# ai4r/Gesture-Generation-from-Trimodal-Context

Measured on AMD Instinct MI355X. Metric: training clips/sec (34-frame, 27-dim pose), post-warm-up GAN iteration, higher is better.
Workload: dtype f32; 1 GPU; multimodal_context GAN training iteration (BASELINE.json configs[1]), epoch > loss_warmup; batch_per_gpu=128, global_batch=128, frames=34, pose_dim=27, audio_samples=36267, n_words=20000, hipgraph=True, parallelism=dp1

## Files before the change

### gesture-generation-from-trimodal-context_amd/_lib.py

```python
import ctypes as C
import os

_HERE = os.path.dirname(os.path.abspath(__file__))
LIB_PATH = os.environ.get("TG_LIB_PATH") or os.path.join(_HERE, "libtrimodal_hip.so")


class Window(C.Structure):
    _fields_ = [("ptr", C.c_void_p), ("batch_stride", C.c_int64), ("row_stride", C.c_int64), ("rows_in", C.c_int32),
                ("rows_out", C.c_int32), ("row_step", C.c_int32), ("shift", C.c_int32), ("dil", C.c_int32),
                ("cw", C.c_int32), ("K", C.c_int32)]


P, I32, I64, F32, U32 = C.c_void_p, C.c_int32, C.c_int64, C.c_float, C.c_uint32
WP = C.POINTER(Window)


class NtProblem(C.Structure):
    _fields_ = [("A", Window), ("Bw", P), ("ldb", I64), ("b_seg_k", I32), ("reserved", I32), ("b_seg_stride", I64), ("bias", P), ("C", P),
                ("c_batch_stride", I64), ("c_row_stride", I64), ("c_rows_out", I32), ("M", I32), ("N", I32), ("act_slope", F32),
                ("accumulate", I32), ("out_scale", P), ("b_planes", P), ("b_plane_stride", I64), ("b_rows", I32), ("b_row0", I32),
                ("gate", P), ("res", P), ("C2", P), ("res_slope", F32), ("drop_site", U32), ("drop_state", P), ("drop_index0", I64),
                ("drop_p", F32), ("reserved4", I32), ("b_planes_kind", I32), ("reserved5", I32), ("b_inv_scale", P), ("a_row_scale", P), ("a_rowmax", P), ("c_rowmax", P), ("c2_rowmax", P), ("a_rowmax_rows", I32), ("reserved6", I32)]


class TnProblem(C.Structure):
    _fields_ = [("dY", P), ("ldy", I64), ("A", Window), ("dW", P), ("ldw", I64), ("M", I32), ("N", I32), ("out_kw", I32), ("reserved", I32),
                ("dbias", P), ("ws", P), ("ws_floats", I64), ("y_colmax", P), ("a_colmax", P)]


class AeStepArgs(C.Structure):
    _fields_ = [("x", P), ("params", P), ("grads", P), ("off", I32 * 44), ("running_mean", P * 8), ("running_var", P * 8),
                ("num_batches_tracked", P * 8), ("ws", P), ("ws_bytes", I64), ("loss", P), ("recon", P), ("feat", P), ("step", P), ("B", I32),
                ("bn_eps", F32), ("momentum", F32), ("last_phase", I32), ("adam_m", P), ("adam_v", P), ("lr", F32), ("beta1", F32), ("beta2", F32), ("adam_eps", F32)]


MAX_GROUP = 8

SIGNATURES = {
    "tg_gemm_nt": [WP, P, I64, P, P, I64, I64, I32, I32, I32, F32, I32, P],
    "tg_gemm_nt_group": [C.POINTER(NtProblem), I32, P],
    "tg_gemm_tn_group": [C.POINTER(TnProblem), I32, P],
    "tg_ae_train_step": [C.POINTER(AeStepArgs), P],
    "tg_split3_planes": [P, I64, I32, I32, P, I32, I64, P],
    "tg_split2h_planes": [P, I64, I32, I32, P, I32, I64, P, P],
    "tg_split2h_planes_tcat": [P, P, I32, I32, P, I32, I64, P, P],
    "tg_win_row_absmax": [WP, I32, P, P],
    "tg_h2_row_scales": [WP, I32, P, P, P],
    "tg_absmax_rows_cols": [P, I64, I32, I32, I32, P, P, P],
    "tg_gemm_tn": [P, I64, WP, P, I64, I32, I32, I32, P, P, I64, P],
    "tg_colsum": [P, I64, I32, I32, P, I32, P],
    "tg_gru_forward": [P, I64, P, P, P, P, P, P, I64, I32, I32, I32, P],
    "tg_gru_backward": [P, P, P, I64, P, P, P, P, I64, P, I32, I32, I32, P],
    "tg_gru_h64_forward": [P, I64, P, P, P, P, P, P, I64, P, P, I32, I32, P],
    "tg_gru_h64_backward": [P, P, P, P, I64, P, P, P, P, I64, I32, I32, P],
    "tg_gru_forward_cluster": [P, I64, P, P, P, P, P, P, I64, P, P, P, I64, I32, I32, I32, P],
    "tg_gru_forward_cluster_rows": [P, I64, P, P, P, P, P, P, I64, P, P, P, I64, I32, I32, I32, I32, I32, P],
    "tg_gru_forward_vec": [P, I64, P, P, P, P, P, P, I64, I32, I32, I32, P],
    "tg_gru_vec1_supported": [I32, I32, P],
    "tg_gru_forward_vec1": [P, P, P, P, P, I64, I32, I32, I32, P],
    "tg_gru_vec_const_supported": [I32, I32, I32, P],
    "tg_gru_forward_vec_const": [P, I64, P, P, P, P, P, P, I64, I32, I32, I32, I32, P],
    "tg_gru_backward_cluster": [P, P, P, P, I64, P, P, P, P, I64, P, I64, I32, I32, I32, P],
    "tg_gru_backward_cluster_stats": [P, P, P, P, I64, P, P, P, P, I64, P, I64, I32, I32, I32, P, I64, P, P, P],
    "tg_bn_train_stats": [P, I32, I32, I32, P, P, P, P, P, P, F32, F32, I32, P],
    "tg_bn_eval_stats": [P, P, I32, F32, P, P, P],
    "tg_bn_train_fused": [P, P, I32, I32, I32, P, P, P, P, P, P, P, F32, F32, F32, I32, P],
    "tg_bn_apply": [P, P, I32, I32, I32, P, P, P, P, F32, P],
    "tg_bn2_train": [P, P, I32, I32, I32, P, I64, P, P, P, P, P, P, P, F32, F32, F32, I32, P],
    "tg_bn2_backward": [P, P, P, I32, I32, I32, P, P, P, P, F32, P, I64, P, P, P],
    "tg_bn_backward": [P, P, P, I32, I32, P, P, P, P, F32, P, P, P, P],
    "tg_wav_front_stats": [P, I64, I32, I32, P, P, I32, I32, I32, P, I64, P, P, P, P, P, P, F32, F32, I32, P],
    "tg_wav_front_apply": [P, I64, I32, I32, P, P, I32, I32, I32, P, P, P, P, F32, P, P, P],
    "tg_wav_front_backward": [P, P, P, I64, I32, I32, P, P, I32, I32, I32, P, P, P, P, F32, P, I64, P, P, P, P, P],
    "tg_wav_front_backward_fused": [P, I32, P, P, P, I64, I32, I32, P, P, I32, I32, I32, P, P, P, P, F32, P, I64, P, P, P, P, P],
    "tg_speaker_fwd": [P, P, I32, P, P, P, P, P, P, P, P, P, P, P, P, I32, P, I64, I32, P, U32, P],
    "tg_speaker_bwd": [P, P, P, P, P, P, P, P, I32, P, P, P, P, P, P, P, P, P, P, I32, P],
    "tg_wav_conv2_wgrad": [P, P, I32, I32, I32, P, I64, P, P, P],
    "tg_out_mlp_compose": [P, P, P, P, I32, I32, I32, I32, P, P, P, P],
    "tg_out_mlp_param_grads": [P, P, P, P, P, I32, I32, I32, I32, P, P, P, P, P],
    "tg_zero": [P, I64, P],
    "tg_permute3_batch": [P, I32, I32, P],
    "tg_add_relu": [P, P, P, I64, P],
    "tg_act_mask_bwd": [P, P, P, F32, P, I64, P],
    "tg_act_mask_bwd2": [P, P, P, P, F32, P, P, I64, P],
    "tg_embed_gather_drop": [P, P, P, I32, I32, I32, F32, P, U32, P],
    "tg_tcn_fwd_fused": [P, P, I64, I32, P, C.POINTER(P), P, P, P, U32, F32, I32, I32, I32, I32, P, P, P, I32, I32, P, I64, P],
    "tg_d_preconv_bwd": [P] * 26 + [I32, P, I64, I32, I32, P],
    "tg_d_preconv_fwd": [P] * 27 + [I64, I32, I32, F32, F32, P],
    "tg_iter_head": [P, P, P, P, P, P, I64, I32, I32, I32, I32, I32, P, P, P, P, I32, P, U32, P, P, P],
    "tg_act_mask_bwd_drop": [P, P, F32, P, U32, I64, F32, P, I64, P],
    "tg_act_mask_bwd2_drop": [P, P, P, F32, P, U32, I64, F32, P, P, I64, P],
    "tg_mul": [P, P, P, I64, P],
    "tg_axpy": [P, P, F32, I32, I64, P],
    "tg_copy2d": [P, I64, P, I64, I32, I32, I32, P],
    "tg_repeat_rows": [P, I64, P, I64, I32, I32, I32, P],
    "tg_sum_rows": [P, I64, P, I64, I32, I32, I32, I32, P],
    "tg_add_halves": [P, P, I32, I32, P],
    "tg_sum_parts": [P, I64, I32, P, I64, P],
    "tg_narrow8_pair": [P, P, P, P, P, I32, I32, P],
    "tg_dup_halves": [P, P, I32, I32, P],
    "tg_make_pre_seq": [P, P, I32, I32, I32, I32, P],
    "tg_embed_gather": [P, P, P, I32, I32, I32, P],
    "tg_assemble_batch": [P, P, P, P, P, P, P, P, P, P, I32, I32, I32, I32, I32, I32, P, P, P, P, P],
    "tg_embed_scatter_add": [P, P, P, I32, I32, I32, P],
    "tg_permute3": [P, P, I32, I32, I32, I32, I32, I32, P],
    "tg_conv_dgrad_pack": [P, P, I32, I32, I32, I32, P],
    "tg_weight_norm_fwd": [P, P, P, I32, I32, I32, P],
    "tg_weight_norm_fwd_batch": [I32, C.POINTER(P), C.POINTER(P), C.POINTER(P), C.POINTER(P), I32, I32, I32, P],
    "tg_weight_norm_bwd": [P, P, P, P, P, I32, I32, I32, P],
    "tg_weight_norm_bwd_batch": [I32, C.POINTER(P), C.POINTER(P), C.POINTER(P), C.POINTER(P), C.POINTER(P), I32, I32, I32, P],
    "tg_rng_advance": [P, P],
    "tg_iter_begin": [P, P, P, P, P],
    "tg_dropout_mask": [P, I64, F32, P, U32, P],
    "tg_dropout_apply": [P, P, P, I64, F32, P, U32, P],
    "tg_normal": [P, I64, P, U32, P],
    "tg_randperm": [P, I32, P, U32, P],
    "tg_gather_i64": [P, P, P, I32, P],
    "tg_reparam_fwd": [P, P, P, P, I64, P],
    "tg_reparam_bwd": [P, P, P, P, P, I64, P],
    "tg_gan_d_loss": [P, P, I32, P, P, P, P],
    "tg_gan_g_loss": [P, P, P, P, P, P, P, P, I32, I32, I32, F32, F32, F32, F32, I32, P, P, P, P, P, P, P],
    "tg_d_head_fwd": [P, P, P, P, P, P, P, P, I32, I32, I32, P],
    "tg_d_head_bwd": [P, P, P, P, P, P, P, P, P, P, I32, I32, I32, P],
    "tg_d_head_step": [P] * 17 + [I32, I32, F32, F32, I32, I32, P],
    "tg_l1_mean": [P, P, I64, P, P],
    "tg_sigmoid": [P, P, I64, P],
    "tg_sigmoid_bwd": [P, P, P, I64, P],
    "tg_window_blend": [P, P, I32, I32, I32, I32, P],
    "tg_window_stage": [P, P, P, P, P, P, I32, I32, I32, I32, P, P, P],
    "tg_spec_stage": [P, P, P, P, P, I32, I32, I32, I32, P, P],
    "tg_utterance_finish": [P, I64, I32, I32, P, I32, I32, I32, I32, P, P, P, P, I64, P],
    "tg_pose_metrics": [P, P, P, I32, I32, I32, P, P],
    "tg_ae_loss": [P, P, I32, I32, I32, P, P, P],
    "tg_counter_inc": [P, P],
    "tg_adam_step": [P, P, P, P, I64, F32, F32, F32, F32, P, P],
    "tg_conv2d_fwd": [P, I32, P, P, P] + [I32] * 12 + [P],
    "tg_conv2d_dgrad": [P, P, P, I32] + [I32] * 12 + [P],
    "tg_conv2d_wgrad_ws_bytes": [I32] * 12 + [P],
    "tg_conv2d_wgrad": [P, P, I32, P, I32, P, I64] + [I32] * 12 + [P],
    "tg_s2g_rows_interp": [P, P, I32, I32, I32, I32, I32, I32, P],
    "tg_s2g_rows_interp_bwd": [P, P, I32, I32, I32, I32, I32, I32, P],
    "tg_s2g_up_add": [P, P, P, I32, I32, I32, I32, P],
    "tg_s2g_up_add_bwd": [P, P, I32, I32, I32, I32, I32, P],
    "tg_s2g_diff": [P, P, I32, I32, I32, P],
    "tg_s2g_diff_bwd": [P, P, I32, I32, I32, I32, P],
    "tg_s2g_mse_const": [P, I64, F32, F32, P, P, P],
    "tg_s2g_l1_grad": [P, P, P, I64, P],
    "tg_logmel_query": [I32, I32, P],
    "tg_logmel": [P, I64, I32, I32, I32, P, I64, P, I64, P, I32, P],
    "tg_pose_resample": [P, I64, I32, P, I64, I32, P, I64, P],
    "tg_clip_windows": [P, I64, I32, P, I64, I32, I32, P, I64, P, P, P, P, P],
# ... 115 lines not shown
```

### gesture-generation-from-trimodal-context_amd/csrc/common.hpp

```cpp
#pragma once
#include <hip/hip_runtime.h>
#include <stdint.h>
#include <stdio.h>
#include <string.h>

#include "../../include/trimodal_hip.h"

typedef float f32x4 __attribute__((ext_vector_type(4)));

namespace tg {

void set_error(const char* fmt, ...);

inline int check_launch(const char* what) {
    hipError_t e = hipGetLastError();
    if (e != hipSuccess) {
        set_error("%s: %s", what, hipGetErrorString(e));
        return 1;
    }
    return 0;
}

#define TG_REQUIRE(cond, ...)              \
    do {                                   \
        if (!(cond)) {                     \
            tg::set_error(__VA_ARGS__);    \
            return 2;                      \
        }                                  \
    } while (0)

extern "C" int tg_get_deterministic(void);
inline bool deterministic() { return tg_get_deterministic() != 0; }

inline bool aligned16(const void* p) { return (reinterpret_cast<uintptr_t>(p) & 15u) == 0; }

inline int cdiv(int64_t a, int64_t b) { return (int)((a + b - 1) / b); }

int zero_async(void* p, size_t bytes, hipStream_t s);

inline int ew_grid(int64_t n, int block = 256, int per_thread = 4) {
    int64_t b = (n + (int64_t)block * per_thread - 1) / ((int64_t)block * per_thread);
    if (b < 1) b = 1;
    if (b > 2048) b = 2048;
    return (int)b;
}

struct Win {
    const float* ptr;
    long bs, rs;
    int rows_in, rows_out, step, shift, dil, cw, K;
};

inline Win to_win(const tg_window* w) {
    Win d;
    d.ptr = w->ptr; d.bs = w->batch_stride; d.rs = w->row_stride; d.rows_in = w->rows_in; d.rows_out = w->rows_out;
    d.step = w->row_step; d.shift = w->shift; d.dil = w->dil; d.cw = w->cw; d.K = w->K;
    return d;
}

constexpr int TG_MAX_GROUP = 8;

struct NtProb {
    Win A;
    const float* Bw;
    long ldb;
    long b_seg_stride;
    int b_seg_k;
    const float* bias;
    const float* mul;
    const uint64_t* drop_state;
    long drop_index0;
    unsigned drop_site;
    float drop_p;
    float* C;
    long cbs, crs;
    int cR, M, N;
    float slope;
    int accumulate;
    int n_nt;
    int vec_c;
    const float* gate;
    const float* res;
    float* C2;
    float res_slope;
    unsigned a_bytes, b_bytes;
    const __bf16* Bpl;
    long bpl_plane;
    int b_slab_rows, b_row0;
    const float* a_scale;
    const float* a_rmax;
    int a_rmax_div;
    const float* b_inv;
    int h2;
    float* c_rmax;
    float* c2_rmax;
};

struct NtGroup {
    int n;
    int wg_begin[TG_MAX_GROUP + 1];
    NtProb p[TG_MAX_GROUP];
};

struct TnProb {
    const float* dY;
    long ldy;
    Win A;
    float* dW;
    long ldw;
    int M, N, rows_per_split, out_kw;
    float* partial;
    float* dbias;
    int vec_y, vec_a, n_nt, n_kt;
    unsigned a_bytes, y_bytes;
    const float* y_cmax;
    const float* a_cmax;
};

struct TnGroup {
    int n;
    int wg_begin[TG_MAX_GROUP + 1];
    TnProb p[TG_MAX_GROUP];
};

template <typename G>
__device__ __forceinline__ int group_find(const G& g, int bid) {
    int i = 0;
#pragma unroll
    for (int q = 1; q < TG_MAX_GROUP; ++q) i += (q < g.n && bid >= g.wg_begin[q]) ? 1 : 0;
    return i;
}

__device__ __forceinline__ int xcd_chunked_id(int bid, int nwg) {
    const int q = nwg >> 3, r = nwg & 7, xcd = bid & 7, pos = bid >> 3;
    return (xcd < r ? xcd * (q + 1) : r * (q + 1) + (xcd - r) * q) + pos;
}

__device__ __forceinline__ float act_fn(float x, float slope) { return x >= 0.f ? x : x * slope; }
__device__ __forceinline__ float sigmoidf_(float x) { return 1.f / (1.f + expf(-x)); }
__device__ __forceinline__ float gate_exp_neg(float x) { return __builtin_amdgcn_exp2f(x * -1.44269504088896341f); }
__device__ __forceinline__ float gate_sigmoid(float x) { return __builtin_amdgcn_rcpf(1.f + gate_exp_neg(x)); }
__device__ __forceinline__ float gate_tanh(float x) {
    const float e = gate_exp_neg(2.f * fabsf(x));
    return copysignf((1.f - e) * __builtin_amdgcn_rcpf(1.f + e), x);
}

__device__ __forceinline__ void split3_bits(float x, unsigned& hi, unsigned& mid, unsigned& lo) {
    hi = __float_as_uint(x) & 0xffff0000u;
    const float r = x - __uint_as_float(hi);
    mid = __float_as_uint(r) & 0xffff0000u;
    lo = __float_as_uint(r - __uint_as_float(mid));
}
__device__ __forceinline__ unsigned pack_hi16(unsigned first, unsigned second) { return __builtin_amdgcn_perm(second, first, 0x07060302u); }

__device__ __host__ __forceinline__ long plane_tiled_off(long r, int c, int rows) { return ((long)(c >> 5) * (rows + 1) + r) * 32 + (c & 31); }

typedef _Float16 tg_f16x2 __attribute__((ext_vector_type(2)));
typedef _Float16 tg_f16x8 __attribute__((ext_vector_type(8)));
__device__ __host__ __forceinline__ int h2_exp_of_bits(unsigned absmax_bits) {
    const int e = (int)((absmax_bits & 0x7fffffffu) >> 23);
    return e < 32 ? 32 : (e > 250 ? 250 : e);
}
__device__ __forceinline__ float h2_scale_of_exp(int e) { return __uint_as_float((unsigned)(268 - e) << 23); }
__device__ __forceinline__ float h2_inv_of_exp(int e) { return __uint_as_float((unsigned)(e - 14) << 23); }
__device__ __forceinline__ float h2_inv_of_scale(float s) { return __uint_as_float(0x7f000000u - __float_as_uint(s)); }
__device__ __forceinline__ void h2_split2(float a, float b, unsigned& hi, unsigned& lo) {
    const tg_f16x2 h = {(_Float16)a, (_Float16)b};
    const float ha = (float)h[0], hb = (float)h[1];
    const tg_f16x2 l = {(_Float16)(a - ha), (_Float16)(b - hb)};
    hi = __builtin_bit_cast(unsigned, h);
    lo = __builtin_bit_cast(unsigned, l);
}
__device__ __forceinline__ unsigned wave_max_u32(unsigned v) {
#pragma unroll
    for (int o = 32; o >= 1; o >>= 1) { const unsigned w = (unsigned)__shfl_xor((int)v, o, 64); v = v > w ? v : w; }
    return v;
}

// ... 32 lines not shown
```

### gesture-generation-from-trimodal-context_amd/csrc/gemm.hip

```cpp
#include <stdlib.h>

#include <type_traits>
#include <utility>

#include "operand_split.hpp"

namespace tg {

template <bool VEC>
__device__ __forceinline__ void load_nt_frags(const Win& A, const long (&a_off)[2], const int (&a_r)[2], const bool (&a_ok)[2],
                                              const float* const (&b_ptr)[2], const bool (&b_ok)[2], int k, int kk, int c,
                                              f32x4 (&fa)[2], f32x4 (&fb)[2]) {
    const int K = A.K;
    if (VEC) {
        const bool inb = k < K;
#pragma unroll
        for (int mt = 0; mt < 2; ++mt) {
            const int sr = a_r[mt] + kk * A.dil;
            const bool ok = a_ok[mt] && inb && sr >= 0 && sr < A.rows_in;
            f32x4 z = {0.f, 0.f, 0.f, 0.f};
            fa[mt] = ok ? *reinterpret_cast<const f32x4*>(A.ptr + a_off[mt] + (long)sr * A.rs + c) : z;
        }
#pragma unroll
        for (int nt = 0; nt < 2; ++nt) {
            f32x4 z = {0.f, 0.f, 0.f, 0.f};
            fb[nt] = (b_ok[nt] && inb) ? *reinterpret_cast<const f32x4*>(b_ptr[nt] + k) : z;
        }
    } else {
#pragma unroll
        for (int v = 0; v < 4; ++v) {
            const int kv = k + v;
            const bool inb = kv < K;
            const int kkv = inb ? kv / A.cw : 0;
            const int cv = kv - kkv * A.cw;
#pragma unroll
            for (int mt = 0; mt < 2; ++mt) {
                const int sr = a_r[mt] + kkv * A.dil;
                const bool ok = a_ok[mt] && inb && sr >= 0 && sr < A.rows_in;
                fa[mt][v] = ok ? A.ptr[a_off[mt] + (long)sr * A.rs + cv] : 0.f;
            }
#pragma unroll
            for (int nt = 0; nt < 2; ++nt) fb[nt][v] = (b_ok[nt] && inb) ? b_ptr[nt][kv] : 0.f;
        }
    }
}

template <bool VEC, int WM, int WN, int NT_RING, int KS = 1>
__global__ __launch_bounds__(256) void gemm_nt_kernel(const NtGroup g) {
    static_assert(KS == 1 || (KS == 4 && WM == 1 && WN == 1 && VEC), "K split: one tile per workgroup, vectorised path");
    const int pi = group_find(g, blockIdx.x);
    const NtProb& pr = g.p[pi];
    const Win A = pr.A;
    const float* __restrict__ Bw = pr.Bw;
    const long ldb = pr.ldb;
    const float* __restrict__ bias = pr.bias;
    const float* __restrict__ mul = pr.mul;
    float* __restrict__ C = pr.C;
    const long cbs = pr.cbs, crs = pr.crs;
    const int cR = pr.cR, M = pr.M, N = pr.N, accumulate = pr.accumulate, n_nt = pr.n_nt;
    const float slope = pr.slope;
    const int lane = threadIdx.x & 63;
    const int wave = threadIdx.x >> 6;
    const int wm = KS > 1 ? 0 : wave / WN, wn = KS > 1 ? 0 : wave % WN;
    const int r16 = lane & 15, kq = lane >> 4;
    const int lid = xcd_chunked_id(blockIdx.x - g.wg_begin[pi], g.wg_begin[pi + 1] - g.wg_begin[pi]);
    const int m_base = (lid / n_nt) * (WM * 32) + wm * 32;
    const int n_base = (lid % n_nt) * (WN * 32) + wn * 32;
    if (m_base >= M || n_base >= N) return;
    const int kslice = KS > 1 ? ((A.K + 16 * KS - 1) / (16 * KS)) * 16 : A.K;
    const int K_beg = KS > 1 ? wave * kslice : 0;
    const int K = KS > 1 ? (A.K < K_beg + kslice ? A.K : K_beg + kslice) : A.K;

    long a_off[2];
    int a_r[2];
    bool a_ok[2];
#pragma unroll
    for (int mt = 0; mt < 2; ++mt) {
        const int m = m_base + mt * 16 + r16;
        a_ok[mt] = m < M;
        const int mm = a_ok[mt] ? m : 0;
        const int b = mm / A.rows_out;
        const int r = mm - b * A.rows_out;
        a_off[mt] = (long)b * A.bs;
        a_r[mt] = r * A.step + A.shift;
    }
    const float* b_ptr[2];
    bool b_ok[2];
#pragma unroll
    for (int nt = 0; nt < 2; ++nt) {
        const int n = n_base + nt * 16 + r16;
        b_ok[nt] = n < N;
        b_ptr[nt] = Bw + (long)(b_ok[nt] ? n : 0) * ldb;
    }

    f32x4 acc[2][2];
#pragma unroll
    for (int i = 0; i < 2; ++i)
#pragma unroll
        for (int j = 0; j < 2; ++j) acc[i][j] = f32x4{0.f, 0.f, 0.f, 0.f};

    if constexpr (VEC) {
        constexpr int R = NT_RING;
        int k = K_beg + 4 * kq;
        int kk = k / A.cw, c = k - (k / A.cw) * A.cw;
        f32x4 ra[R][2], rb[R][2];
        unsigned rm[R];
        auto load = [&](auto set_c) {
            constexpr int j = decltype(set_c)::value;
            const bool inb = k < K;
            unsigned m = 0u;
#pragma unroll
            for (int mt = 0; mt < 2; ++mt) {
                const int sr = a_r[mt] + kk * A.dil;
                const bool ok = a_ok[mt] && inb && sr >= 0 && sr < A.rows_in;
                ra[j][mt] = *reinterpret_cast<const f32x4*>(ok ? A.ptr + a_off[mt] + (long)sr * A.rs + c : A.ptr);
                m |= ok ? (1u << mt) : 0u;
            }
#pragma unroll
            for (int nt = 0; nt < 2; ++nt) {
                const bool ok = b_ok[nt] && inb;
                rb[j][nt] = *reinterpret_cast<const f32x4*>(ok ? b_ptr[nt] + k : Bw);
                m |= ok ? (4u << nt) : 0u;
            }
            rm[j] = m;
            k += 16;
            c += 16;
            while (c >= A.cw) { c -= A.cw; ++kk; }
        };
        static_for<R>([&](auto j) { load(j); });
        for (int k0 = K_beg; k0 < K; k0 += 16 * R) {
            static_for<R>([&](auto jc) {
                constexpr int j = decltype(jc)::value;
                {
                    const f32x4 z = {0.f, 0.f, 0.f, 0.f};
                    f32x4 fa[2], fb[2];
#pragma unroll
                    for (int i = 0; i < 2; ++i) {
                        fa[i] = (rm[j] >> i) & 1u ? ra[j][i] : z;
                        fb[i] = (rm[j] >> (2 + i)) & 1u ? rb[j][i] : z;
                    }
#pragma unroll
                    for (int v = 0; v < 4; ++v)
#pragma unroll
                        for (int mt = 0; mt < 2; ++mt)
#pragma unroll
                            for (int nt = 0; nt < 2; ++nt)
                                acc[mt][nt] = __builtin_amdgcn_mfma_f32_16x16x4f32(fa[mt][v], fb[nt][v], acc[mt][nt], 0, 0, 0);
                    if constexpr (R >= 8) { if (k0 + 16 * R < K) load(jc); }
                    else load(jc);
                }
            });
        }
    } else {
        int k = 4 * kq;
        f32x4 fa[2], fb[2], na[2], nb[2];
        load_nt_frags<VEC>(A, a_off, a_r, a_ok, b_ptr, b_ok, k, 0, k, fa, fb);
        for (int k0 = 0; k0 < K; k0 += 16) {
            const bool more = k0 + 16 < K;
            if (more) {
                k += 16;
                load_nt_frags<VEC>(A, a_off, a_r, a_ok, b_ptr, b_ok, k, 0, k, na, nb);
            }
#pragma unroll
            for (int v = 0; v < 4; ++v)
#pragma unroll
                for (int mt = 0; mt < 2; ++mt)
#pragma unroll
                    for (int nt = 0; nt < 2; ++nt)
                        acc[mt][nt] = __builtin_amdgcn_mfma_f32_16x16x4f32(fa[mt][v], fb[nt][v], acc[mt][nt], 0, 0, 0);
            if (more) {
#pragma unroll
                for (int i = 0; i < 2; ++i) { fa[i] = na[i]; fb[i] = nb[i]; }
            }
        }
    }

    if constexpr (KS > 1) {
        __shared__ f32x4 red[KS - 1][4][64];
        if (wave > 0) {
#pragma unroll
            for (int mt = 0; mt < 2; ++mt)
#pragma unroll
                for (int nt = 0; nt < 2; ++nt) red[wave - 1][mt * 2 + nt][lane] = acc[mt][nt];
        }
        __syncthreads();
        if (wave > 0) return;
#pragma unroll
        for (int q = 0; q < KS - 1; ++q)
#pragma unroll
            for (int mt = 0; mt < 2; ++mt)
#pragma unroll
                for (int nt = 0; nt < 2; ++nt) acc[mt][nt] += red[q][mt * 2 + nt][lane];
    }

    long off[2][4][2];
    bool okc[2][4][2];
    float bv[2] = {0.f, 0.f}, mv[2][4][2], cv[2][4][2];
#pragma unroll
    for (int nt = 0; nt < 2; ++nt) {
        const int col = n_base + nt * 16 + r16;
        if (bias) bv[nt] = bias[col < N ? col : 0];
    }
#pragma unroll
    for (int mt = 0; mt < 2; ++mt)
#pragma unroll
        for (int i = 0; i < 4; ++i) {
            const int row = m_base + mt * 16 + kq * 4 + i;
            const int rr = row < M ? row : 0;
            const int cb = rr / cR;
            const int cr = rr - cb * cR;
#pragma unroll
            for (int nt = 0; nt < 2; ++nt) {
                const int col = n_base + nt * 16 + r16;
                okc[mt][i][nt] = row < M && col < N;
                off[mt][i][nt] = okc[mt][i][nt] ? (long)cb * cbs + (long)cr * crs + col : 0;
                if (mul) mv[mt][i][nt] = mul[off[mt][i][nt]];
                if (accumulate) cv[mt][i][nt] = C[off[mt][i][nt]];
            }
        }
#pragma unroll
    for (int mt = 0; mt < 2; ++mt)
#pragma unroll
        for (int i = 0; i < 4; ++i)
#pragma unroll
            for (int nt = 0; nt < 2; ++nt) {
                float v = act_fn(acc[mt][nt][i] + bv[nt], slope);
                if (mul) v *= mv[mt][i][nt];
                if (accumulate) v += cv[mt][i][nt];
                if (okc[mt][i][nt]) C[off[mt][i][nt]] = v;
            }
}

template <int TM, int TN, int BK = 16>
__global__ __launch_bounds__(256) void gemm_nt_big_kernel(const NtGroup g) {
    const int pi = group_find(g, blockIdx.x);
    const NtProb& pr = g.p[pi];
    const Win A = pr.A;
    const float* __restrict__ Bw = pr.Bw;
    const long ldb = pr.ldb, b_seg_stride = pr.b_seg_stride;
    const int b_seg_k = pr.b_seg_k;
    const float* __restrict__ bias = pr.bias;
    const float* __restrict__ mul = pr.mul;
    float* __restrict__ C = pr.C;
    const long cbs = pr.cbs, crs = pr.crs;
    const int cR = pr.cR, M = pr.M, N = pr.N, accumulate = pr.accumulate, n_nt = pr.n_nt;
    const float slope = pr.slope;
    constexpr int BM = 32 * TM, BN = 32 * TN;
    constexpr int PPR = BK / 4;
    constexpr int RPP = 256 / PPR;
    constexpr int NPA = (BM + RPP - 1) / RPP;
    constexpr int NPB = (BN + RPP - 1) / RPP;
    constexpr int LD = BK + 4;
    __shared__ __attribute__((aligned(16))) float as[2][BM][LD];
    __shared__ __attribute__((aligned(16))) float bs[2][BN][LD];
    const int t = threadIdx.x;
    const int lane = t & 63, wave = t >> 6;
    const int wm = wave >> 1, wn = wave & 1;
    const int r16 = lane & 15, kq = lane >> 4;
    const int lid = xcd_chunked_id(blockIdx.x - g.wg_begin[pi], g.wg_begin[pi + 1] - g.wg_begin[pi]);
    const int m0 = (lid / n_nt) * BM, n0 = (lid % n_nt) * BN;
    if (m0 >= M) return;
    const int K = A.K;

    const int srow = t / PPR, sk = 4 * (t % PPR);
    long a_off[NPA];
    int a_r[NPA];
    bool a_ok[NPA];
#pragma unroll
    for (int i = 0; i < NPA; ++i) {
        const int m = m0 + srow + RPP * i;
        a_ok[i] = (srow + RPP * i < BM) && m < M;
        const int mm = a_ok[i] ? m : 0;
        const int b = mm / A.rows_out;
        const int r = mm - b * A.rows_out;
        a_off[i] = (long)b * A.bs;
        a_r[i] = r * A.step + A.shift;
    }
    const float* b_ptr[NPB];
    bool b_ok[NPB];
#pragma unroll
    for (int i = 0; i < NPB; ++i) {
        const int n = n0 + srow + RPP * i;
        b_ok[i] = (srow + RPP * i < BN) && n < N;
        b_ptr[i] = Bw + (long)(b_ok[i] ? n : 0) * ldb;
    }
    int kk = sk / A.cw, c = sk - (sk / A.cw) * A.cw;
    int bsg = sk / b_seg_k, bc = sk - (sk / b_seg_k) * b_seg_k;

    f32x4 ga[NPA], gb[NPB];
    auto fetch = [&](int k0) {
        const int k = k0 + sk;
        const bool inb = k < K;
#pragma unroll
        for (int i = 0; i < NPA; ++i) {
            const int sr = a_r[i] + kk * A.dil;
            const bool ok = a_ok[i] && inb && sr >= 0 && sr < A.rows_in;
            f32x4 z = {0.f, 0.f, 0.f, 0.f};
            ga[i] = ok ? *reinterpret_cast<const f32x4*>(A.ptr + a_off[i] + (long)sr * A.rs + c) : z;
        }
#pragma unroll
        for (int i = 0; i < NPB; ++i) {
            f32x4 z = {0.f, 0.f, 0.f, 0.f};
            gb[i] = (b_ok[i] && inb) ? *reinterpret_cast<const f32x4*>(b_ptr[i] + bsg * b_seg_stride + bc) : z;
        }
        c += BK;
        while (c >= A.cw) { c -= A.cw; ++kk; }
        bc += BK;
        while (bc >= b_seg_k) { bc -= b_seg_k; ++bsg; }
    };

    f32x4 acc[TM][TN];
#pragma unroll
    for (int i = 0; i < TM; ++i)
// ... 266 lines not shown
    float s = 0.f;
    if (n < N)
        for (int m = m_begin + rp; m < m_end; m += 4) s += X[(long)m * ldx + n];
    red[rp][cidx] = s;
    __syncthreads();
    if (rp == 0 && n < N) atomicAdd(&out[n], red[0][cidx] + red[1][cidx] + red[2][cidx] + red[3][cidx]);
}

template <int CW>
__global__ __launch_bounds__(1024) void colsum_det_kernel(const float* __restrict__ X, long ldx, int M, int N, float* __restrict__ out, int accumulate) {
    constexpr int RL = 1024 / CW;
    __shared__ double red[RL][CW];
    const int cidx = threadIdx.x % CW, rp = threadIdx.x / CW;
    const int n = blockIdx.x * CW + cidx;
    double s = 0.0;
    if (n < N) {
        int m = rp;
        for (; m + 7 * RL < M; m += 8 * RL) {
            float v[8];
#pragma unroll
            for (int u = 0; u < 8; ++u) v[u] = X[(long)(m + RL * u) * ldx + n];
#pragma unroll
            for (int u = 0; u < 8; ++u) s += v[u];
        }
        for (; m < M; m += RL) s += X[(long)m * ldx + n];
    }
    red[rp][cidx] = s;
    __syncthreads();
    if (rp == 0 && n < N) {
        double t = 0.0;
        for (int q = 0; q < RL; ++q) t += red[q][cidx];
        out[n] = (accumulate ? out[n] : 0.f) + (float)t;
    }
}

}

using namespace tg;

extern "C" int tg_get_math_mode(void);
int tg_gemm_nt_split_launch(NtGroup& g, hipStream_t s);
int tg_gemm_tn_split_launch(const TnGroup& g, int total_wgs, int tnw, int tkw, hipStream_t s);
bool tg_gemm_tn_mw_plan(TnGroup& g, int* splits_out, int* grid, const long* ws_floats);
int tg_gemm_tn_mw_launch(const TnGroup& g, int grid, int splits, hipStream_t s);
int tg_gemm_tn_mw_reduce_launch(const TnGroup& g, const int* splits, hipStream_t s);
static bool use_split_path() {
    static int x3 = -1;
    if (x3 < 0) {
        const char* e = getenv("TG_GEMM_X3");
        x3 = (e && e[0] == '0') ? 0 : 1;
    }
    return x3 == 1 || tg_get_math_mode() == 1;
}

static int check_window(const tg_window* w, const char* who) {
    TG_REQUIRE(w && w->ptr, "%s: null window", who);
    TG_REQUIRE(w->K > 0 && w->cw > 0 && w->K % w->cw == 0, "%s: K=%d must be a positive multiple of cw=%d", who, w->K, w->cw);
    TG_REQUIRE(w->rows_out > 0 && w->rows_in > 0, "%s: rows_out/rows_in must be positive", who);
    return 0;
}

static bool nt_vec(const NtProb& p) {
    const Win& w = p.A;
    return (w.cw % 4 == 0) && (w.K % 4 == 0) && (w.bs % 4 == 0) && (w.rs % 4 == 0) && aligned16(w.ptr) && (p.ldb % 4 == 0) && aligned16(p.Bw) &&
           (p.b_seg_k % 4 == 0) && (p.b_seg_stride % 4 == 0);
}
static bool nt_has_ext(const NtProb& p) { return p.gate != nullptr || p.res != nullptr || p.drop_state != nullptr; }
static int nt_family(const NtProb& p) {
    if (nt_vec(p) && p.N >= 48 && p.M >= 1024 && p.A.K >= 64) return 0;
    return p.N <= 32 ? 1 : 2;
}

static int nt_layout(NtGroup& g, int bm, int bn) {
    int wg = 0;
    for (int i = 0; i < g.n; ++i) {
        g.p[i].n_nt = cdiv(g.p[i].N, bn);
        g.wg_begin[i] = wg;
        wg += (cdiv(g.p[i].M, bm) * g.p[i].n_nt + 7) / 8 * 8;
    }
    for (int i = g.n; i <= TG_MAX_GROUP; ++i) g.wg_begin[i] = wg;
    return wg;
}

static int nt_launch(NtGroup& g, hipStream_t s) {
    const int fam = nt_family(g.p[0]);
    bool vec = true;
    for (int i = 0; i < g.n; ++i) {
        TG_REQUIRE(nt_family(g.p[i]) == fam, "tg_gemm_nt_group: problem %d does not fit the kernel family of problem 0 (M=%d N=%d K=%d)", i,
                   g.p[i].M, g.p[i].N, g.p[i].A.K);
        vec = vec && nt_vec(g.p[i]);
        TG_REQUIRE(fam == 0 || g.p[i].b_seg_k == g.p[i].A.K, "tg_gemm_nt: K-concatenated weights need the big-product path (problem %d)", i);
    }
    if (fam == 0 && use_split_path()) return tg_gemm_nt_split_launch(g, s);
    for (int i = 0; i < g.n; ++i)
        TG_REQUIRE(!g.p[i].c_rmax && !g.p[i].c2_rmax, "tg_gemm_nt: c_rowmax / c2_rowmax are outputs of the mover-wave kernel only (tg_gemm_nt_kernel_plan == 2; problem %d)", i);
    for (int i = 0; i < g.n; ++i)
        TG_REQUIRE(!nt_has_ext(g.p[i]), "tg_gemm_nt: gate / res / C2 / regenerated dropout need the big-product split path (tg_gemm_nt_ext_supported; problem %d)", i);
    if (fam == 0) {
        int Mx = 0, Nx = 0;
        for (int i = 0; i < g.n; ++i) { Mx = Mx > g.p[i].M ? Mx : g.p[i].M; Nx = Nx > g.p[i].N ? Nx : g.p[i].N; }
        const NtTile tl = nt_pick_tile(Mx * g.n, Nx);
        const dim3 grid(nt_layout(g, 32 * tl.tm, 32 * tl.tn));
#define TG_NT_BIG(TM_, TN_) hipLaunchKernelGGL((gemm_nt_big_kernel<TM_, TN_>), grid, dim3(256), 0, s, g)
        if (tl.tm == 4 && tl.tn == 4) TG_NT_BIG(4, 4);
        else if (tl.tm == 4 && tl.tn == 3) TG_NT_BIG(4, 3);
        else if (tl.tm == 4 && tl.tn == 2) TG_NT_BIG(4, 2);
        else if (tl.tm == 2 && tl.tn == 2) TG_NT_BIG(2, 2);
        else TG_NT_BIG(2, 1);
#undef TG_NT_BIG
    } else {
        int Kx = 0;
        for (int i = 0; i < g.n; ++i) Kx = Kx > g.p[i].A.K ? Kx : g.p[i].A.K;
        const int wgs = fam == 1 ? nt_layout(g, 128, 32) : nt_layout(g, 64, 64);
        const dim3 grid(wgs);
        const bool deep = wgs < 1024 && Kx >= 256;
        if (fam == 1 && vec && wgs < 256 && Kx >= 256) {
            const dim3 grid4(nt_layout(g, 32, 32));
            hipLaunchKernelGGL((gemm_nt_kernel<true, 1, 1, 2, 4>), grid4, dim3(256), 0, s, g);
            return check_launch("tg_gemm_nt");
        }
        int Mmax = 0;
        for (int i = 0; i < g.n; ++i) Mmax = Mmax > g.p[i].M ? Mmax : g.p[i].M;
        if (fam == 2 && vec && wgs <= 64 && Kx >= 256 && Mmax <= 576) {
            const dim3 grid4(nt_layout(g, 32, 32));
            if (Kx <= 640) hipLaunchKernelGGL((gemm_nt_kernel<true, 1, 1, 10, 4>), grid4, dim3(256), 0, s, g);
            else hipLaunchKernelGGL((gemm_nt_kernel<true, 1, 1, 2, 4>), grid4, dim3(256), 0, s, g);
            return check_launch("tg_gemm_nt");
        }
        if (fam == 1) {
            if (vec && deep) hipLaunchKernelGGL((gemm_nt_kernel<true, 4, 1, 4>), grid, dim3(256), 0, s, g);
            else if (vec)    hipLaunchKernelGGL((gemm_nt_kernel<true, 4, 1, 1>), grid, dim3(256), 0, s, g);
            else             hipLaunchKernelGGL((gemm_nt_kernel<false, 4, 1, 1>), grid, dim3(256), 0, s, g);
        } else {
            if (vec && deep) hipLaunchKernelGGL((gemm_nt_kernel<true, 2, 2, 4>), grid, dim3(256), 0, s, g);
            else if (vec)    hipLaunchKernelGGL((gemm_nt_kernel<true, 2, 2, 1>), grid, dim3(256), 0, s, g);
            else             hipLaunchKernelGGL((gemm_nt_kernel<false, 2, 2, 1>), grid, dim3(256), 0, s, g);
        }
    }
    return check_launch("tg_gemm_nt");
}

static int nt_fill(NtProb& p, const tg_gemm_nt_problem& q, int idx) {
    if (int e = check_window(&q.A, "tg_gemm_nt")) return e;
    TG_REQUIRE(q.Bw && q.C, "tg_gemm_nt: null pointer (problem %d)", idx);
    TG_REQUIRE(q.M > 0 && q.N > 0 && q.c_rows_out > 0, "tg_gemm_nt: bad sizes M=%d N=%d (problem %d)", q.M, q.N, idx);
    const int seg = q.b_seg_k > 0 ? q.b_seg_k : q.A.K;
    TG_REQUIRE(q.A.K % seg == 0 && q.ldb >= seg, "tg_gemm_nt: weight segments of %d do not tile K=%d / ldb=%ld (problem %d)", seg, q.A.K,
               (long)q.ldb, idx);
    p.A = to_win(&q.A);
    p.Bw = q.Bw; p.ldb = (long)q.ldb; p.b_seg_k = seg; p.b_seg_stride = q.b_seg_k > 0 ? (long)q.b_seg_stride : 0;
    TG_REQUIRE(q.drop_state == nullptr || (q.out_scale == nullptr && q.drop_index0 >= 0 && q.drop_index0 % 4 == 0 && q.drop_p >= 0.f && q.drop_p < 1.f),
               "tg_gemm_nt: regenerated dropout (problem %d) excludes out_scale and needs drop_index0 %% 4 == 0, 0 <= drop_p < 1", idx);
    p.drop_state = q.drop_state; p.drop_index0 = (long)q.drop_index0; p.drop_site = q.drop_site; p.drop_p = q.drop_p;
    p.bias = q.bias; p.mul = q.out_scale; p.C = q.C; p.cbs = (long)q.c_batch_stride; p.crs = (long)q.c_row_stride; p.cR = q.c_rows_out;
    p.M = q.M; p.N = q.N; p.slope = q.act_slope; p.accumulate = q.accumulate; p.n_nt = 0;
    p.a_bytes = p.b_bytes = 0;
    p.Bpl = nullptr; p.bpl_plane = 0; p.b_slab_rows = 0; p.b_row0 = 0;
    p.h2 = 0; p.a_scale = nullptr; p.a_rmax = nullptr; p.b_inv = nullptr; p.a_rmax_div = 1;
    p.c_rmax = q.c_rowmax; p.c2_rmax = q.c2_rowmax;
    TG_REQUIRE(!q.c2_rowmax || q.C2, "tg_gemm_nt: c2_rowmax without C2 (problem %d)", idx);
    if (q.b_planes) {
        const int64_t kp = ((int64_t)q.A.K + 31) / 32 * 32;
        TG_REQUIRE(q.b_rows >= q.N && q.b_row0 >= 0 && q.b_row0 + (int64_t)q.N <= q.b_rows && aligned16(q.b_planes) &&
                       q.b_plane_stride >= ((int64_t)q.b_rows + 1) * kp && q.b_plane_stride % 8 == 0 && ((int64_t)q.b_rows + 1) * kp < (1LL << 30),
                   "tg_gemm_nt: bad weight planes (problem %d): one weight matrix, its N=%d rows inside the buffer's %d, plane stride >= (rows + 1) * K "
                   "rounded up to 32, 16-byte aligned", idx, q.N, q.b_rows);
        p.Bpl = reinterpret_cast<const __bf16*>(q.b_planes); p.bpl_plane = (long)q.b_plane_stride; p.b_slab_rows = q.b_rows + 1; p.b_row0 = q.b_row0;
        if (q.b_planes_kind == 1) {
            TG_REQUIRE(q.b_inv_scale && ((q.a_row_scale != nullptr) != (q.a_rowmax != nullptr)) && aligned16(q.b_inv_scale) && q.b_row0 % 4 == 0,
                       "tg_gemm_nt: fp16 x 2 weight planes (problem %d) need b_inv_scale (16-byte aligned), exactly one of a_row_scale / a_rowmax and b_row0 %% 4 == 0", idx);
            TG_REQUIRE(!q.a_rowmax || q.A.K <= 2 * q.A.cw, "tg_gemm_nt: a_rowmax serves windows of at most two taps (problem %d: %d); pass a_row_scale (tg_h2_row_scales)",
                       idx, q.A.K / q.A.cw);
            TG_REQUIRE(q.a_rowmax_rows >= 0 && (int64_t)cdiv(q.M, q.A.rows_out) * q.A.rows_in < (1LL << 31), "tg_gemm_nt: bad a_rowmax_rows=%d (problem %d)", q.a_rowmax_rows, idx);
            p.h2 = 1; p.a_scale = q.a_row_scale; p.a_rmax = q.a_rowmax; p.b_inv = q.b_inv_scale; p.a_rmax_div = q.a_rowmax_rows > 0 ? q.a_rowmax_rows : 1;
        } else TG_REQUIRE(q.b_planes_kind == 0, "tg_gemm_nt: b_planes_kind=%d (problem %d): 0 (bf16 x 3) or 1 (fp16 x 2)", q.b_planes_kind, idx);
    }
    TG_REQUIRE((q.res == nullptr) == (q.C2 == nullptr), "tg_gemm_nt: res and C2 go together (problem %d)", idx);
    p.gate = q.gate; p.res = q.res; p.C2 = q.C2; p.res_slope = q.res_slope;
    p.vec_c = (q.N % 4 == 0) && (q.c_batch_stride % 4 == 0) && (q.c_row_stride % 4 == 0) && aligned16(q.C) &&
              (q.bias == nullptr || aligned16(q.bias)) && (q.out_scale == nullptr || aligned16(q.out_scale)) &&
              (q.gate == nullptr || aligned16(q.gate)) && (q.res == nullptr || (aligned16(q.res) && aligned16(q.C2)));
    return 0;
}


extern "C" int32_t tg_gemm_nt_family(const tg_gemm_nt_problem* problem) {
    NtProb p;
    if (!problem || nt_fill(p, *problem, 0)) return -1;
    return nt_family(p);
}

extern "C" int32_t tg_gemm_nt_ext_supported(const tg_gemm_nt_problem* problem) {
    NtProb p;
    if (!problem || nt_fill(p, *problem, 0)) return 0;
    return nt_family(p) == 0 && use_split_path() ? 1 : 0;
}

bool tg_gemm_nt_mw_eligible(NtGroup& g, int* tm, int* tn);
extern "C" int32_t tg_gemm_nt_kernel_plan(const tg_gemm_nt_problem* problems, int32_t n, int32_t* tile_m, int32_t* tile_n) {
    if (!problems || n < 1 || n > TG_MAX_GROUP) return -1;
    NtGroup g;
    g.n = n;
    for (int i = 0; i < n; ++i)
        if (nt_fill(g.p[i], problems[i], i)) return -1;
    for (int i = n; i < TG_MAX_GROUP; ++i) g.p[i] = g.p[0];
    const int fam = nt_family(g.p[0]);
    for (int i = 0; i < n; ++i)
        if (nt_family(g.p[i]) != fam) return -1;
    if (fam != 0 || !use_split_path()) return 0;
    int tm = 0, tn = 0;
    if (!tg_gemm_nt_mw_eligible(g, &tm, &tn)) return 1;
    if (tile_m) *tile_m = 32 * tm;
    if (tile_n) *tile_n = 32 * tn;
    return 2;
}

extern "C" int tg_gemm_nt_group(const tg_gemm_nt_problem* problems, int32_t n, void* stream) {
    TG_REQUIRE(problems && n >= 1 && n <= TG_MAX_GROUP, "tg_gemm_nt_group: 1..%d problems", TG_MAX_GROUP);
    NtGroup g;
    g.n = n;
    for (int i = 0; i < n; ++i)
        if (int e = nt_fill(g.p[i], problems[i], i)) return e;
    for (int i = n; i < TG_MAX_GROUP; ++i) g.p[i] = g.p[0];
    return nt_launch(g, (hipStream_t)stream);
}

extern "C" int tg_gemm_nt(const tg_window* A, const float* Bw, int64_t ldb, const float* bias, float* C,
                          int64_t c_batch_stride, int64_t c_row_stride, int32_t c_rows_out, int32_t M, int32_t N,
                          float act_slope, int32_t accumulate, void* stream) {
    TG_REQUIRE(A, "tg_gemm_nt: null window");
    tg_gemm_nt_problem q = {};
    q.A = *A; q.Bw = Bw; q.ldb = ldb; q.b_seg_k = 0; q.b_seg_stride = 0; q.bias = bias; q.C = C; q.c_batch_stride = c_batch_stride;
    q.c_row_stride = c_row_stride; q.c_rows_out = c_rows_out; q.M = M; q.N = N; q.act_slope = act_slope; q.accumulate = accumulate;
    q.out_scale = nullptr; q.reserved = 0;
    TG_REQUIRE(ldb >= A->K, "tg_gemm_nt: ldb=%ld < K=%d", (long)ldb, A->K);
    return tg_gemm_nt_group(&q, 1, stream);
}

static void tn_plan(int M, int tiles, bool two_pass, int* splits_out, int* rows_out) {
    int splits = cdiv(M, 320);
    if (splits < cdiv(640, tiles)) splits = cdiv(640, tiles);
    if (two_pass) {
        const int by_len = cdiv(M, 512);
        if (splits < by_len) splits = by_len;
    }
    const int max_splits = cdiv(M, 64);
    if (splits > max_splits) splits = max_splits;
    if (splits < 1) splits = 1;
    if (splits > 65535) splits = 65535;
    int rows = cdiv(M, splits);
    rows = ((rows + 31) / 32) * 32;
    *rows_out = rows;
    *splits_out = cdiv(M, rows);
}

static void launch_tn_reduce(const float* partial, int splits, int N, int K, int cw, int out_kw, float* dW, long ldw, hipStream_t s) {
    const long total = (long)N * K;
    if (splits >= 512) {
        const long blocks = total > 4096 ? 4096 : total;
        hipLaunchKernelGGL(tn_reduce_kernel_t<256>, dim3((int)blocks), dim3(256), 0, s, partial, splits, N, K, cw, out_kw, dW, ldw);
    } else {
        long blocks = (total + 15) / 16;
        if (blocks > 4096) blocks = 4096;
        hipLaunchKernelGGL(tn_reduce_kernel_t<16>, dim3((int)blocks), dim3(256), 0, s, partial, splits, N, K, cw, out_kw, dW, ldw);
    }
}

extern "C" int64_t tg_gemm_tn_ws_floats(int32_t M, int32_t N, int32_t K) {
    int splits, rows;
    tn_plan(M, cdiv(N, 64) * cdiv(K, 64), true, &splits, &rows);
    return (int64_t)splits * N * K;
}

static int tn_fill(TnProb& p, const tg_gemm_tn_problem& q, int idx, int group_tiles, int bn, int bk, int* splits_out) {
    if (int e = check_window(&q.A, "tg_gemm_tn")) return e;
    TG_REQUIRE(q.dY && q.dW && q.M > 0 && q.N > 0 && q.ldy >= q.N && q.ldw >= q.A.K, "tg_gemm_tn: bad arguments (problem %d)", idx);
    TG_REQUIRE(q.out_kw == 0 || q.out_kw * q.A.cw == q.A.K, "tg_gemm_tn: out_kw=%d must be 0 or K/cw (problem %d)", q.out_kw, idx);
    p.A = to_win(&q.A);
    int splits, rows_per_split;
    tn_plan(q.M, cdiv(q.N, bn) * cdiv(p.A.K, bk), q.ws != nullptr, &splits, &rows_per_split);
    if (q.ws == nullptr && group_tiles > cdiv(q.N, bn) * cdiv(p.A.K, bk)) {
        constexpr int target_wgs = 768;
        constexpr int target_wgs22 = 2000;
        int s2 = cdiv(bn == 64 ? target_wgs22 : target_wgs, group_tiles);
        const int cap = cdiv(q.M, 256);
        if (s2 > cap) s2 = cap;
        if (s2 < 1) s2 = 1;
        if (s2 < splits) {
            int rows = cdiv(q.M, s2);
            rows = ((rows + 31) / 32) * 32;
            rows_per_split = rows;
            splits = cdiv(q.M, rows);
        }
    }
    TG_REQUIRE(q.ws == nullptr || q.ws_floats >= (int64_t)splits * q.N * p.A.K, "tg_gemm_tn: workspace too small (%ld < %ld floats, problem %d)",
               (long)q.ws_floats, (long)splits * q.N * p.A.K, idx);
    p.dY = q.dY; p.ldy = (long)q.ldy; p.dW = q.dW; p.ldw = (long)q.ldw; p.M = q.M; p.N = q.N; p.rows_per_split = rows_per_split;
    p.out_kw = q.out_kw; p.partial = q.ws; p.dbias = q.dbias;
    TG_REQUIRE((q.y_colmax == nullptr) == (q.a_colmax == nullptr) && aligned16(q.y_colmax) && aligned16(q.a_colmax),
               "tg_gemm_tn: y_colmax and a_colmax go together, 16-byte aligned (problem %d)", idx);
    p.y_cmax = q.y_colmax; p.a_cmax = q.a_colmax;
    p.vec_y = (q.ldy % 4 == 0) && aligned16(q.dY);
    p.vec_a = (p.A.cw % 4 == 0) && (p.A.bs % 4 == 0) && (p.A.rs % 4 == 0) && aligned16(p.A.ptr);
    p.n_nt = cdiv(q.N, bn); p.n_kt = cdiv(p.A.K, bk);
    *splits_out = splits;
    return 0;
// ... 114 lines not shown
```

### gesture-generation-from-trimodal-context_amd/csrc/gemm_split.hip

```cpp
#include "operand_split.hpp"
#include "tr_image.hpp"
#include <stdlib.h>
#include <type_traits>

namespace tg {

constexpr int SP_LD = 32;

template <int TM, int TN, int SPLITS, int DB, int RING = 1, int OCC = 1, int ABL = 0, bool FAST = false>
__global__ __launch_bounds__(256, OCC) void gemm_nt_split_kernel(const NtGroup g) {
    const int pi = group_find(g, blockIdx.x);
    const NtProb& pr = g.p[pi];
    const Win A = pr.A;
    const float* __restrict__ Bw = pr.Bw;
    const long ldb = pr.ldb, b_seg_stride = pr.b_seg_stride;
    const int b_seg_k = pr.b_seg_k;
    const float* __restrict__ bias = pr.bias;
    const float* __restrict__ mul = pr.mul;
    const uint64_t* __restrict__ drop = pr.drop_state;
    const float* __restrict__ gate = pr.gate;
    const float* __restrict__ res = pr.res;
    float* __restrict__ C2 = pr.C2;
    const float slope2 = pr.res_slope;
    float* __restrict__ C = pr.C;
    const long cbs = pr.cbs, crs = pr.crs;
    const int cR = pr.cR, M = pr.M, N = pr.N, accumulate = pr.accumulate, n_nt = pr.n_nt;
    const float slope = pr.slope;
    constexpr int BM = 32 * TM, BN = 32 * TN;
    constexpr int NPA = BM / 32, NPB = BN / 32;
    constexpr int NS = SPLITS;
    constexpr int NB = DB ? 2 : 1;
    constexpr int CLD = BN + 4;
    constexpr int OPER_BYTES = NB * NS * (BM + BN) * SP_LD * 2, CT_BYTES = BM * CLD * 4;
    __shared__ __attribute__((aligned(16))) unsigned char smem[OPER_BYTES > CT_BYTES ? OPER_BYTES : CT_BYTES];
    typedef __bf16 (*lds_t)[NS][BM + BN][SP_LD];
    const lds_t lds = reinterpret_cast<lds_t>(smem);
    const int t = threadIdx.x, lane = t & 63, wave = t >> 6;
    const int wm = wave >> 1, wn = wave & 1;
    const int r16 = lane & 15, kq = lane >> 4;
    const int lid = xcd_chunked_id(blockIdx.x - g.wg_begin[pi], g.wg_begin[pi + 1] - g.wg_begin[pi]);
    const int m0 = (lid / n_nt) * BM, n0 = (lid % n_nt) * BN;
    if (m0 >= M) return;
    const int K = A.K;

    const int sp = 4 * (t & 7), sr0 = t >> 3;
    const int sp_w = sp ^ slab_swz(sr0), fcol = (8 * kq) ^ slab_swz(r16);
    long a_off[NPA];
    int a_r[NPA];
    bool a_ok[NPA];
    unsigned a_base[NPA], b_base[NPB];
#pragma unroll
    for (int q = 0; q < NPA; ++q) {
        const int m = m0 + sr0 + 32 * q;
        a_ok[q] = m < M;
        const int mm = a_ok[q] ? m : (FAST ? M - 1 : 0);
        const int b = mm / A.rows_out;
        a_off[q] = (long)b * A.bs;
        a_r[q] = (mm - b * A.rows_out) * A.step + A.shift;
        a_base[q] = (unsigned)((a_off[q] + (long)a_r[q] * A.rs) * 4);
    }
    const float* b_ptr[NPB];
    bool b_ok[NPB];
#pragma unroll
    for (int q = 0; q < NPB; ++q) {
        const int n = n0 + sr0 + 32 * q;
        b_ok[q] = n < N;
        b_ptr[q] = Bw + (long)(b_ok[q] ? n : (FAST ? N - 1 : 0)) * ldb;
        b_base[q] = (unsigned)((long)(b_ok[q] ? n : N - 1) * ldb * 4);
    }
    int kk = sp / A.cw, c = sp - (sp / A.cw) * A.cw;
    int bsg = sp / b_seg_k, bc = sp - (sp / b_seg_k) * b_seg_k;
    unsigned ka = (unsigned)(((long)kk * A.dil * A.rs + c) * 4), kb = (unsigned)(((long)bsg * b_seg_stride + bc) * 4);
    const unsigned ka_wrap = (unsigned)(((long)A.dil * A.rs - A.cw) * 4), kb_wrap = (unsigned)((b_seg_stride - b_seg_k) * 4);
    const char* const a_bytes = reinterpret_cast<const char*>(A.ptr);
    const char* const b_bytes = reinterpret_cast<const char*>(Bw);

    f32x4 ga[RING][NPA], gb[RING][NPB];
    unsigned ga_ok[RING], gb_ok[RING];
    auto fetch = [&](auto set_c, int k0) {
        constexpr int set = decltype(set_c)::value;
        const int k = k0 + sp;
        const bool inb = k < K;
        unsigned ma = 0u, mb = 0u;
        if constexpr (FAST) {
            const unsigned oa = inb ? ka : 0u, ob = inb ? kb : 0u;
#pragma unroll
            for (int q = 0; q < NPA; ++q) ga[set][q] = *reinterpret_cast<const f32x4*>(a_bytes + (a_base[q] + oa));
#pragma unroll
            for (int q = 0; q < NPB; ++q) gb[set][q] = *reinterpret_cast<const f32x4*>(b_bytes + (b_base[q] + ob));
            ga_ok[set] = gb_ok[set] = inb ? ~0u : 0u;
            c += 32; ka += 128u;
            if (c >= A.cw) { c -= A.cw; ka += ka_wrap; }
// ... 100 lines not shown
    using tail_t = std::true_type;
    using full_t = std::false_type;
    fetch(set0{}, 0);
    if constexpr (RING == 2) {
        if (32 < K) fetch(set1{}, 32);
        int k0 = 0;
        if constexpr (FAST) {
            for (; k0 + 64 <= K; k0 += 64) {
                slab(set0{}, k0, full_t{});
                slab(set1{}, k0 + 32, full_t{});
            }
            if (k0 + 32 <= K) {
                slab(set0{}, k0, full_t{});
                if (k0 + 32 < K) slab(set1{}, k0 + 32, tail_t{});
            } else if (k0 < K) slab(set0{}, k0, tail_t{});
        } else {
            for (; k0 < K; k0 += 64) {
                slab(set0{}, k0, tail_t{});
                if (k0 + 32 < K) slab(set1{}, k0 + 32, tail_t{});
            }
        }
    } else {
        int k0 = 0;
        if constexpr (FAST) {
            for (; k0 + 32 <= K; k0 += 32) slab(set0{}, k0, full_t{});
            if (k0 < K) slab(set0{}, k0, tail_t{});
        } else {
            for (; k0 < K; k0 += 32) slab(set0{}, k0, tail_t{});
        }
    }

    const int vec_c = pr.vec_c;
    if (vec_c) {
        float* ct = reinterpret_cast<float*>(smem);
        __syncthreads();
#pragma unroll
        for (int i = 0; i < TM; ++i)
#pragma unroll
            for (int q = 0; q < 4; ++q)
#pragma unroll
                for (int j = 0; j < TN; ++j)
                    ct[(wm * (16 * TM) + i * 16 + kq * 4 + q) * CLD + wn * (16 * TN) + j * 16 + r16] = acc[i][j][q];
        __syncthreads();
        constexpr int C4 = BN / 4, NP = BM * C4 / 256, CH = 4;
        static_assert(BM * C4 % 256 == 0, "whole pieces per thread");
        const f32x4 z4 = {0.f, 0.f, 0.f, 0.f};
#pragma unroll
        for (int p0 = 0; p0 < NP; p0 += CH) {
            f32x4 bv[CH], mv[CH], cv[CH], gv[CH], rv[CH];
            long o[CH];
            bool ok[CH];
#pragma unroll
            for (int u = 0; u < CH; ++u) {
                if (p0 + u >= NP) continue;
                const int idx = t + 256 * (p0 + u);
                const int rl = idx / C4, c4 = idx - rl * C4;
                const int row = m0 + rl, col = n0 + 4 * c4;
                ok[u] = row < M && col < N;
                const int cb = row / cR;
                const int cr = row - cb * cR;
                o[u] = ok[u] ? (long)cb * cbs + (long)cr * crs + col : 0;
                bv[u] = bias ? *reinterpret_cast<const f32x4*>(bias + (ok[u] ? col : 0)) : z4;
                if (mul) mv[u] = *reinterpret_cast<const f32x4*>(mul + o[u]);
                else if (drop) mv[u] = dropout_scale4(drop, pr.drop_site, pr.drop_p, (unsigned long)(pr.drop_index0 + o[u]) >> 2);
                if (gate) gv[u] = *reinterpret_cast<const f32x4*>(gate + o[u]);
                if (res) rv[u] = *reinterpret_cast<const f32x4*>(res + o[u]);
                if (accumulate) cv[u] = *reinterpret_cast<const f32x4*>(C + o[u]);
            }
#pragma unroll
            for (int u = 0; u < CH; ++u) {
                if (p0 + u >= NP) continue;
                const int idx = t + 256 * (p0 + u);
                const int rl = idx / C4, c4 = idx - rl * C4;
                f32x4 v = *reinterpret_cast<const f32x4*>(&ct[rl * CLD + 4 * c4]) + bv[u];
#pragma unroll
                for (int q = 0; q < 4; ++q) v[q] = act_fn(v[q], slope);
                if (mul || drop) v *= mv[u];
                if (gate) {
#pragma unroll
                    for (int q = 0; q < 4; ++q) v[q] = gv[u][q] > 0.f ? v[q] : 0.f;
                }
                if (accumulate) v += cv[u];
                if (ok[u]) *reinterpret_cast<f32x4*>(C + o[u]) = v;
                if (res) {
                    f32x4 w = v + rv[u];
#pragma unroll
                    for (int q = 0; q < 4; ++q) w[q] = act_fn(w[q], slope2);
                    if (ok[u]) *reinterpret_cast<f32x4*>(C2 + o[u]) = w;
                }
            }
        }
        return;
    }
#pragma unroll
    for (int i = 0; i < TM; ++i) {
#pragma unroll
        for (int q = 0; q < 4; ++q) {
            const int row = m0 + wm * (16 * TM) + i * 16 + kq * 4 + q;
            if (row >= M) continue;
            const int cb = row / cR;
            const int cr = row - cb * cR;
            const long ro = (long)cb * cbs + (long)cr * crs;
            float* crow = C + ro;
            const float* mrow = mul ? mul + ro : nullptr;
#pragma unroll
            for (int j = 0; j < TN; ++j) {
                const int col = n0 + wn * (16 * TN) + j * 16 + r16;
                if (col >= N) continue;
                float v = acc[i][j][q];
                if (bias) v += bias[col];
                v = act_fn(v, slope);
                if (mrow) v *= mrow[col];
                if (gate) v = gate[ro + col] > 0.f ? v : 0.f;
                if (accumulate) v += crow[col];
                crow[col] = v;
                if (res) C2[ro + col] = act_fn(v + res[ro + col], slope2);
            }
        }
    }
}

template <int TNW, int TKW>
__global__ __launch_bounds__(256) void gemm_tn_split_kernel(const TnGroup g) {
    const int pi = group_find(g, blockIdx.x);
    const TnProb& pr = g.p[pi];
    const float* __restrict__ dY = pr.dY;
    const long ldy = pr.ldy, ldw = pr.ldw;
    const Win A = pr.A;
    float* __restrict__ dW = pr.dW;
    const int M = pr.M, N = pr.N, rows_per_split = pr.rows_per_split, out_kw = pr.out_kw;
    float* __restrict__ partial = pr.partial;
    float* __restrict__ dbias = pr.dbias;
    const int n_nt = pr.n_nt, n_kt = pr.n_kt;
    constexpr int MR = 32;
    constexpr int BN = 32 * TNW, BK = 32 * TKW;
    using YI = TrImage<BN>;
    using XI = TrImage<BK>;
    constexpr int LDN = YI::LD, LDK = XI::LD;
    constexpr int PY = BN / 4, PX = BK / 4;
    __shared__ __attribute__((aligned(16))) __bf16 ys[2][3][MR][LDN];
    __shared__ __attribute__((aligned(16))) __bf16 xs[2][3][MR][LDK];
    const int t = threadIdx.x;
    const int lane = t & 63, wave = t >> 6;
    const int r16 = lane & 15, kq = lane >> 4;
    const int wn = wave >> 1, wk = wave & 1;
    const int lid = xcd_chunked_id(blockIdx.x - g.wg_begin[pi], g.wg_begin[pi + 1] - g.wg_begin[pi]);
    const int tn_n = lid % n_nt, tn_k = (lid / n_nt) % n_kt, tn_s = lid / (n_nt * n_kt);
    const int n0 = tn_n * BN, k0 = tn_k * BK;
    const int K = A.K;
    const int m_begin = tn_s * rows_per_split;
    if (m_begin >= M) return;
    const int m_end = min(M, m_begin + rows_per_split);

    int yrow[TNW], ycol[TNW], ypos[TNW];
    bool y_ok[TNW];
#pragma unroll
    for (int i = 0; i < TNW; ++i) {
        const int p = t + 256 * i;
        yrow[i] = p / PY;
        ycol[i] = 4 * (p - yrow[i] * PY);
        y_ok[i] = n0 + ycol[i] < N;
        ypos[i] = YI::at(yrow[i], ycol[i]);
    }
    int xrow[TKW], xcol[TKW], xpos[TKW], a_off[TKW], a_tapd[TKW], mb[TKW], mr[TKW];
    bool a_ok[TKW];
#pragma unroll
    for (int i = 0; i < TKW; ++i) {
        const int p = t + 256 * i;
        xrow[i] = p / PX;
        xcol[i] = 4 * (p - xrow[i] * PX);
        xpos[i] = XI::at(xrow[i], xcol[i]);
// ... 92 lines not shown
    fetch(set1{}, m_begin + MR);
    for (int m0 = m_begin; m0 < m_end; m0 += 2 * MR) {
        slab(set0{}, m0 + 2 * MR);
        slab(set1{}, m0 + 3 * MR);
    }

#pragma unroll
    for (int nt = 0; nt < TNW; ++nt)
#pragma unroll
        for (int kt = 0; kt < TKW; ++kt)
#pragma unroll
            for (int i = 0; i < 4; ++i) {
                const int n = n0 + wn * (16 * TNW) + nt * 16 + kq * 4 + i;
                const int kcol = k0 + wk * (16 * TKW) + kt * 16 + r16;
                if (n < N && kcol < K && partial) {
                    partial[((long)tn_s * N + n) * K + kcol] = acc[nt][kt][i];
                } else if (n < N && kcol < K) {
                    const long off = out_kw > 0 ? (long)(kcol % A.cw) * out_kw + kcol / A.cw : (long)kcol;
                    atomicAdd(&dW[(long)n * ldw + off], acc[nt][kt][i]);
                }
            }
    if (want_bias) {
        float (*bs)[BN + 4] = reinterpret_cast<float (*)[BN + 4]>(&ys[0][0][0][0]);
        static_assert(sizeof(float) * MR * (BN + 4) <= sizeof(ys), "bias scratch fits the dY image");
        __syncthreads();
#pragma unroll
        for (int i = 0; i < TNW; ++i) *reinterpret_cast<f32x4*>(&bs[yrow[i]][ycol[i]]) = bsum[i];
        __syncthreads();
        if (t < BN && n0 + t < N) {
            float sacc = 0.f;
#pragma unroll
            for (int r = 0; r < MR; ++r) sacc += bs[r][t];
            atomicAdd(&dbias[n0 + t], sacc);
        }
    }
}

}

using namespace tg;

static int g_math_mode = 0;

extern "C" int tg_set_math_mode(int32_t mode) {
    TG_REQUIRE(mode == 0 || mode == 1, "tg_set_math_mode: mode must be 0 (fp32-accurate) or 1 (bf16 operands)");
    g_math_mode = mode;
    return 0;
}

extern "C" int tg_get_math_mode(void) { return g_math_mode; }

static int g_deterministic = 0;
extern "C" int tg_set_deterministic(int32_t on) { g_deterministic = on ? 1 : 0; return 0; }
extern "C" int tg_get_deterministic(void) { return g_deterministic; }

static bool nt_fast_ok(const NtProb& p) {
    const Win& A = p.A;
    if (A.cw < 32 || p.b_seg_k < 32 || A.K < 64 || A.cw % 4 != 0 || p.b_seg_k % 4 != 0 || A.K % A.cw != 0 || A.K % p.b_seg_k != 0) return false;
    const int taps = A.K / A.cw, segs = A.K / p.b_seg_k;
    if (A.rows_out <= 0 || p.M % A.rows_out != 0) return false;
    const long r_lo = (A.step >= 0 ? 0 : (long)(A.rows_out - 1) * A.step) + A.shift + (A.dil >= 0 ? 0 : (long)(taps - 1) * A.dil);
    const long r_hi = (A.step >= 0 ? (long)(A.rows_out - 1) * A.step : 0) + A.shift + (A.dil >= 0 ? (long)(taps - 1) * A.dil : 0);
    if (r_lo < 0 || r_hi >= A.rows_in) return false;
    if (A.bs < 0 || A.rs < 0 || p.ldb < 0 || p.b_seg_stride < 0) return false;
    const long batches = p.M / A.rows_out;
    const long a_max = (batches - 1) * A.bs + r_hi * A.rs + A.cw;
    const long b_max = (long)(p.N - 1) * p.ldb + (long)(segs - 1) * p.b_seg_stride + p.b_seg_k;
    return a_max < (1l << 29) && b_max < (1l << 29);
}

struct SplitTile { int tm, tn, db; };
static SplitTile split_pick_tile(int M, int N) {
    auto wgs = [&](int bm, int bn) { return (long)cdiv(M, bm) * cdiv(N, bn); };
    auto waste = [&](int bn) { return cdiv(N, bn) * bn - N; };
    if (wgs(128, 96) >= 512 && waste(96) <= waste(64) + 32) return {4, 3, 0};
    if (wgs(128, 64) >= 384) return {4, 2, 0};
    if (wgs(64, 96) >= 256 && waste(96) <= waste(64) + 32) return {2, 3, 1};
    return {2, 2, 1};
}

bool tg_gemm_nt_mw_eligible(NtGroup& g, int* tm, int* tn);
int tg_gemm_nt_mw_launch(NtGroup& g, int tm, int tn, int splits, hipStream_t s);

int tg_gemm_nt_split_launch(NtGroup& g, hipStream_t s) {
    {
        int tm = 0, tn = 0;
        if (tg_gemm_nt_mw_eligible(g, &tm, &tn)) {
            TG_REQUIRE(!(g.p[0].h2 && g_math_mode == 1), "tg_gemm_nt: fp16 x 2 weight planes belong to the fp32-accurate mode, not to the bf16 tier");
            return tg_gemm_nt_mw_launch(g, tm, tn, g_math_mode == 1 ? 1 : 3, s);
        }
    }
    for (int i = 0; i < g.n; ++i)
        TG_REQUIRE(!g.p[i].c_rmax && !g.p[i].c2_rmax, "tg_gemm_nt: c_rowmax / c2_rowmax are outputs of the mover-wave kernel only (tg_gemm_nt_kernel_plan == 2; problem %d)", i);
    for (int i = 0; i < g.n; ++i)
        TG_REQUIRE(g.p[i].drop_state == nullptr || g.p[i].vec_c, "tg_gemm_nt: regenerated dropout needs a vectorisable C (N %% 4 == 0, strides %% 4 == 0, "
                   "16-byte aligned; problem %d)", i);
    int Mx = 0, Nx = 0;
    for (int i = 0; i < g.n; ++i) { Mx = Mx > g.p[i].M ? Mx : g.p[i].M; Nx = Nx > g.p[i].N ? Nx : g.p[i].N; }
    const SplitTile tl = split_pick_tile(Mx * g.n, Nx);
    const int bm = 32 * tl.tm, bn = 32 * tl.tn;
    int wg = 0;
    for (int i = 0; i < g.n; ++i) {
        g.p[i].n_nt = cdiv(g.p[i].N, bn);
        g.wg_begin[i] = wg;
        wg += (cdiv(g.p[i].M, bm) * g.p[i].n_nt + 7) / 8 * 8;
    }
    for (int i = g.n; i <= TG_MAX_GROUP; ++i) g.wg_begin[i] = wg;
    const dim3 grid(wg);
#define TG_SPLIT(TM_, TN_, SP_, DB_)                                                                                   \
    do {                                                                                                               \
        if (TM_ == 4 && SP_ == 3) hipLaunchKernelGGL((gemm_nt_split_kernel<TM_, TN_, SP_, DB_, 1, (TM_ == 4 && SP_ == 3) ? (TN_ == 3 ? 3 : 4) : 1>), grid, dim3(256), 0, s, g); \
        else hipLaunchKernelGGL((gemm_nt_split_kernel<TM_, TN_, SP_, DB_, 1>), grid, dim3(256), 0, s, g);              \
    } while (0)
#define TG_SPLIT_MENU(SP_)                                              \
    do {                                                                \
        if (tl.tm == 4 && tl.tn == 3) TG_SPLIT(4, 3, SP_, 0);           \
        else if (tl.tm == 4 && tl.tn == 2) TG_SPLIT(4, 2, SP_, 0);      \
        else if (tl.tm == 2 && tl.tn == 3) TG_SPLIT(2, 3, SP_, 1);      \
        else TG_SPLIT(2, 2, SP_, 1);                                    \
    } while (0)
    static const int fast_on = [] { const char* e = getenv("TG_NT_FAST"); return e ? atoi(e) : 1; }();
    bool fast = fast_on != 0 && g_math_mode == 0;
    for (int i = 0; i < g.n && fast; ++i) fast = nt_fast_ok(g.p[i]);
    if (fast) {
#define TG_FAST(TM_, TN_, DB_, R_, O_) hipLaunchKernelGGL((gemm_nt_split_kernel<TM_, TN_, 3, DB_, R_, O_, 0, true>), grid, dim3(256), 0, s, g)
        if (tl.tm == 4 && tl.tn == 3) TG_FAST(4, 3, 0, 1, 3);
        else if (tl.tm == 4 && tl.tn == 2) TG_FAST(4, 2, 0, 1, 4);
        else if (tl.tm == 2 && tl.tn == 3) TG_FAST(2, 3, 1, 1, 1);
        else TG_FAST(2, 2, 1, 1, 1);
#undef TG_FAST
        return check_launch("tg_gemm_nt(split, fast addressing)");
    }
#ifdef TG_LAB_ABLATE
    {
        const char* e = getenv("TG_NT_ABL");
        const int abl = e ? atoi(e) : 0;
        if (abl && tl.tm == 4 && tl.tn == 3 && g_math_mode == 0) {
#define TG_ABL(A_) case A_: hipLaunchKernelGGL((gemm_nt_split_kernel<4, 3, 3, 0, 1, 3, A_>), grid, dim3(256), 0, s, g); return check_launch("tg_gemm_nt(split, ablated)")
            switch (abl) { TG_ABL(1); TG_ABL(2); TG_ABL(3); TG_ABL(4); TG_ABL(5); TG_ABL(7); TG_ABL(8); TG_ABL(9); TG_ABL(11); TG_ABL(15); default: break; }
#undef TG_ABL
        }
    }
#endif
    if (g_math_mode == 1) TG_SPLIT_MENU(1);
    else TG_SPLIT_MENU(3);
#undef TG_SPLIT_MENU
#undef TG_SPLIT
    return check_launch("tg_gemm_nt(split)");
}

int tg_gemm_tn_split_launch(const TnGroup& g, int total_wgs, int tnw, int tkw, hipStream_t s) {
#define TG_TN(TNW_, TKW_) hipLaunchKernelGGL((gemm_tn_split_kernel<TNW_, TKW_>), dim3(total_wgs), dim3(256), 0, s, g)
    if (tnw == 2 && tkw == 2) TG_TN(2, 2);
    else if (tnw == 4 && tkw == 4) TG_TN(4, 4);
    else if (tnw == 4 && tkw == 5) TG_TN(4, 5);
    else if (tnw == 5 && tkw == 5) TG_TN(5, 5);
    else if (tnw == 4 && tkw == 2) TG_TN(4, 2);
    else TG_REQUIRE(false, "tg_gemm_tn(split): no %d x %d tile", tnw, tkw);
#undef TG_TN
    return check_launch("tg_gemm_tn(split)");
}
```

### gesture-generation-from-trimodal-context_amd/csrc/norm.hip

```cpp
#include "common.hpp"

namespace tg {

__global__ __launch_bounds__(256) void bn_stats_kernel(const float* __restrict__ x, int rows_per_group, int C, double* __restrict__ ws) {
    __shared__ double sh[2][256];
    const int g = blockIdx.y;
    const int rpi = 256 / C;
    const int c = threadIdx.x % C, rsub = threadIdx.x / C;
    const float* xg = x + (long)g * rows_per_group * C;
    double s = 0.0, ss = 0.0;
    if (rsub < rpi)
        for (long r = (long)blockIdx.x * rpi + rsub; r < rows_per_group; r += (long)gridDim.x * rpi) {
            const float v = xg[r * C + c];
            s += v;
            ss += (double)v * v;
        }
    sh[0][threadIdx.x] = s;
    sh[1][threadIdx.x] = ss;
    __syncthreads();
    if (threadIdx.x < C) {
        double a = 0.0, b = 0.0;
        for (int q = 0; q < rpi; ++q) { a += sh[0][q * C + c]; b += sh[1][q * C + c]; }
        atomicAdd(&ws[((long)g * 2 + 0) * C + c], a);
        atomicAdd(&ws[((long)g * 2 + 1) * C + c], b);
// ... 324 lines not shown
        if (dgamma) dgamma[threadIdx.x] += (float)sh_b[threadIdx.x];
    }
    double m1[4], m2[4];
#pragma unroll
    for (int q = 0; q < 4; ++q) { m1[q] = sh_a[c0 + q] / (double)rows; m2[q] = sh_b[c0 + q] / (double)rows; }
    f32x4* dx4 = reinterpret_cast<f32x4*>(dx);
#pragma unroll 4
    for (long i = threadIdx.x; i < total4; i += BN_SMALL_THREADS) {
        const f32x4 xv = x4[i], dv = dy4[i];
        f32x4 o;
#pragma unroll
        for (int q = 0; q < 4; ++q) {
            const float xh = (xv[q] - mu[q]) * rs[q];
            const float z = xh * ga[q] + be[q];
            const float dz = dv[q] * (z > 0.f ? 1.f : slope);
            o[q] = (float)((double)(ga[q] * rs[q]) * ((double)dz - m1[q] - (double)xh * m2[q]));
        }
        dx4[i] = o;
    }
}

__global__ __launch_bounds__(256) void bn2_partial_kernel(const float* __restrict__ x, const float* __restrict__ dy, long rows_per_group, int C,
                                                          const float* __restrict__ mean, const float* __restrict__ rstd,
                                                          const float* __restrict__ gamma, const float* __restrict__ beta, float slope,
                                                          double* __restrict__ part, int det) {
    __shared__ double sh[2][256];
    __shared__ double sh_det[256][8];
    const int g = blockIdx.y, P = gridDim.x;
    const long total4 = rows_per_group * C / 4;
    const long base4 = (long)g * total4;
    const long i0 = (long)blockIdx.x * 256 + threadIdx.x, step = (long)P * 256;
    const int c0 = (int)((i0 * 4) % C);
    if ((int)threadIdx.x < C) { sh[0][threadIdx.x] = 0.0; sh[1][threadIdx.x] = 0.0; }
    __syncthreads();
    const f32x4* x4 = reinterpret_cast<const f32x4*>(x) + base4;
    double s[4] = {0.0, 0.0, 0.0, 0.0}, ss[4] = {0.0, 0.0, 0.0, 0.0};
    if (dy == nullptr) {
#pragma unroll 4
        for (long i = i0; i < total4; i += step) {
            const f32x4 v = x4[i];
#pragma unroll
            for (int q = 0; q < 4; ++q) { s[q] += v[q]; ss[q] += (double)v[q] * v[q]; }
        }
    } else {
        const f32x4* dy4 = reinterpret_cast<const f32x4*>(dy) + base4;
        float mu[4], rs[4], ga[4], be[4];
#pragma unroll
        for (int q = 0; q < 4; ++q) { mu[q] = mean[g * C + c0 + q]; rs[q] = rstd[g * C + c0 + q]; ga[q] = gamma[c0 + q]; be[q] = beta[c0 + q]; }
#pragma unroll 4
        for (long i = i0; i < total4; i += step) {
            const f32x4 xv = x4[i], dv = dy4[i];
#pragma unroll
            for (int q = 0; q < 4; ++q) {
                const float xh = (xv[q] - mu[q]) * rs[q];
                const float z = xh * ga[q] + be[q];
                const float dz = dv[q] * (z > 0.f ? 1.f : slope);
                s[q] += dz;
                ss[q] += (double)dz * xh;
            }
        }
    }
    if (det) {
#pragma unroll
        for (int q = 0; q < 4; ++q) { sh_det[threadIdx.x][q] = s[q]; sh_det[threadIdx.x][4 + q] = ss[q]; }
        __syncthreads();
        if ((int)threadIdx.x < C) {
            const int c = threadIdx.x;
            double a = 0.0, b = 0.0;
            for (int t = c >> 2; t < 256; t += C / 4) { a += sh_det[t][c & 3]; b += sh_det[t][4 + (c & 3)]; }
            sh[0][c] = a; sh[1][c] = b;
        }
    } else {
#pragma unroll
        for (int q = 0; q < 4; ++q) { atomicAdd(&sh[0][c0 + q], s[q]); atomicAdd(&sh[1][c0 + q], ss[q]); }
    }
    __syncthreads();
    if ((int)threadIdx.x < C) {
        double* o = part + (((long)g * P + blockIdx.x) * 2) * C;
        o[threadIdx.x] = sh[0][threadIdx.x];
        o[C + threadIdx.x] = sh[1][threadIdx.x];
    }
}

__device__ __forceinline__ void bn2_totals(const double* __restrict__ part, int g, int P, int C, double (*tot)[256], double (*sl)[256]) {
    const int S = 256 / C;
    const int c = threadIdx.x % C, sidx = threadIdx.x / C;
    double a = 0.0, b = 0.0;
    if (sidx < S) {
#pragma unroll 8
        for (int p = sidx; p < P; p += S) {
            const double* o = part + (((long)g * P + p) * 2) * C;
            a += o[c];
            b += o[C + c];
        }
    }
    sl[0][threadIdx.x] = a;
    sl[1][threadIdx.x] = b;
    __syncthreads();
    if ((int)threadIdx.x < C) {
        double ta = 0.0, tb = 0.0;
        for (int q = 0; q < S; ++q) { ta += sl[0][q * C + c]; tb += sl[1][q * C + c]; }
        tot[0][c] = ta;
        tot[1][c] = tb;
    }
    __syncthreads();
}

__global__ __launch_bounds__(256) void bn2_reduce_kernel(const double* __restrict__ part, int P, int C, double* __restrict__ out) {
    __shared__ double tot[2][256], sl[2][256];
    bn2_totals(part, blockIdx.x, P, C, tot, sl);
    if ((int)threadIdx.x < C) {
        out[((long)blockIdx.x * 2) * C + threadIdx.x] = tot[0][threadIdx.x];
        out[((long)blockIdx.x * 2 + 1) * C + threadIdx.x] = tot[1][threadIdx.x];
    }
}

__global__ __launch_bounds__(256) void bn2_fwd_apply_kernel(const float* __restrict__ x, float* __restrict__ y, long rows_per_group, int C, int groups,
                                                            const double* __restrict__ part, int P, float* __restrict__ mean, float* __restrict__ rstd,
                                                            float* __restrict__ rmean, float* __restrict__ rvar, int64_t* __restrict__ nbt,
                                                            const float* __restrict__ gamma, const float* __restrict__ beta, float slope, float eps,
                                                            float momentum, int repeats) {
    __shared__ double tot[2][256], sl[2][256];
    __shared__ float s_mean[256], s_rstd[256];
    const int g = blockIdx.y;
    const double n = (double)rows_per_group;
    if (blockIdx.x == 0 && g == 0) {
        float rm = 0.f, rv = 0.f;
        if ((int)threadIdx.x < C) { rm = rmean ? rmean[threadIdx.x] : 0.f; rv = rvar ? rvar[threadIdx.x] : 0.f; }
        for (int gg = 0; gg < groups; ++gg) {
            bn2_totals(part, gg, P, C, tot, sl);
            if ((int)threadIdx.x < C) {
                const int c = threadIdx.x;
                const double m = tot[0][c] / n;
                double var = tot[1][c] / n - m * m;
                if (var < 0.0) var = 0.0;
                const double unbiased = rows_per_group > 1 ? var * n / (n - 1.0) : var;
                for (int q = 0; q < repeats; ++q) {
                    rm = (1.f - momentum) * rm + momentum * (float)m;
                    rv = (1.f - momentum) * rv + momentum * (float)unbiased;
                }
            }
            __syncthreads();
        }
        if ((int)threadIdx.x < C) {
            if (rmean) rmean[threadIdx.x] = rm;
            if (rvar) rvar[threadIdx.x] = rv;
        }
        if (threadIdx.x == 0 && nbt) *nbt += (int64_t)groups * repeats;
    }
    bn2_totals(part, g, P, C, tot, sl);
    if ((int)threadIdx.x < C) {
        const int c = threadIdx.x;
        const double m = tot[0][c] / n;
        double var = tot[1][c] / n - m * m;
        if (var < 0.0) var = 0.0;
        const float mf = (float)m, rs = (float)(1.0 / sqrt(var + (double)eps));
        s_mean[c] = mf; s_rstd[c] = rs;
        if (blockIdx.x == 0) { mean[g * C + c] = mf; rstd[g * C + c] = rs; }
    }
    __syncthreads();
    if (y == nullptr) return;
    const long total4 = rows_per_group * C / 4;
    const long i0 = (long)blockIdx.x * 256 + threadIdx.x, step = (long)gridDim.x * 256;
    const int c0 = (int)((i0 * 4) % C);
    float mu[4], rs[4], ga[4], be[4];
#pragma unroll
    for (int q = 0; q < 4; ++q) { mu[q] = s_mean[c0 + q]; rs[q] = s_rstd[c0 + q]; ga[q] = gamma[c0 + q]; be[q] = beta[c0 + q]; }
    const f32x4* x4 = reinterpret_cast<const f32x4*>(x) + (long)g * total4;
    f32x4* y4 = reinterpret_cast<f32x4*>(y) + (long)g * total4;
#pragma unroll 4
    for (long i = i0; i < total4; i += step) {
        const f32x4 v = x4[i];
        f32x4 o;
#pragma unroll
        for (int q = 0; q < 4; ++q) o[q] = act_fn((v[q] - mu[q]) * rs[q] * ga[q] + be[q], slope);
        y4[i] = o;
    }
}

__global__ __launch_bounds__(256) void bn2_bwd_apply_kernel(const float* __restrict__ dy, const float* __restrict__ x, float* __restrict__ dx,
                                                            long rows_per_group, int C, int groups, const double* __restrict__ part, int P,
                                                            const float* __restrict__ mean, const float* __restrict__ rstd,
                                                            const float* __restrict__ gamma, const float* __restrict__ beta, float slope,
                                                            float* __restrict__ dgamma, float* __restrict__ dbeta) {
    __shared__ double tot[2][256], sl[2][256];
    const int g = blockIdx.y;
    if (blockIdx.x == 0 && g == 0 && (dgamma || dbeta)) {
        double a = 0.0, b = 0.0;
        for (int gg = 0; gg < groups; ++gg) {
            bn2_totals(part, gg, P, C, tot, sl);
            if ((int)threadIdx.x < C) { a += tot[0][threadIdx.x]; b += tot[1][threadIdx.x]; }
            __syncthreads();
        }
        if ((int)threadIdx.x < C) {
            if (dbeta) dbeta[threadIdx.x] += (float)a;
            if (dgamma) dgamma[threadIdx.x] += (float)b;
        }
    }
    bn2_totals(part, g, P, C, tot, sl);
    const long total4 = rows_per_group * C / 4;
    const long i0 = (long)blockIdx.x * 256 + threadIdx.x, step = (long)gridDim.x * 256;
    const int c0 = (int)((i0 * 4) % C);
    const double inv_n = 1.0 / (double)rows_per_group;
    float mu[4], rs[4], ga[4], be[4];
    double m1[4], m2[4];
#pragma unroll
    for (int q = 0; q < 4; ++q) {
        mu[q] = mean[g * C + c0 + q]; rs[q] = rstd[g * C + c0 + q]; ga[q] = gamma[c0 + q]; be[q] = beta[c0 + q];
        m1[q] = tot[0][c0 + q] * inv_n; m2[q] = tot[1][c0 + q] * inv_n;
    }
    const f32x4* x4 = reinterpret_cast<const f32x4*>(x) + (long)g * total4;
    const f32x4* dy4 = reinterpret_cast<const f32x4*>(dy) + (long)g * total4;
    f32x4* dx4 = reinterpret_cast<f32x4*>(dx) + (long)g * total4;
#pragma unroll 2
    for (long i = i0; i < total4; i += step) {
        const f32x4 xv = x4[i], dv = dy4[i];
        f32x4 o;
#pragma unroll
        for (int q = 0; q < 4; ++q) {
            const float xh = (xv[q] - mu[q]) * rs[q];
            const float z = xh * ga[q] + be[q];
            const float dz = dv[q] * (z > 0.f ? 1.f : slope);
            o[q] = (float)((double)(ga[q] * rs[q]) * ((double)dz - m1[q] - (double)xh * m2[q]));
        }
        dx4[i] = o;
    }
}

inline bool bn_vec_ok(int C, long elems) { return C >= 4 && C <= 256 && C % 4 == 0 && 1024 % C == 0 && elems % 4 == 0; }

}

using namespace tg;

extern "C" int32_t tg_bn_fused_supported(int32_t rows, int32_t C, int32_t groups) {
    return C >= 4 && C <= 256 && C % 4 == 0 && 4096 % C == 0 && groups > 0 && rows > 0 && rows % groups == 0 && (long)rows * C <= BN_SMALL_MAX &&
           ((long)(rows / groups) * C) % 4 == 0;
}

extern "C" int tg_bn_train_fused(const float* x, float* y, int32_t rows, int32_t C, int32_t groups, float* mean, float* rstd,
                                 float* running_mean, float* running_var, int64_t* num_batches_tracked, const float* gamma,
                                 const float* beta, float act_slope, float eps, float momentum, int32_t repeats, void* stream) {
    TG_REQUIRE(x && mean && rstd && repeats >= 1 && (y == nullptr || (gamma && beta)), "tg_bn_train_fused: null pointer / repeats < 1");
    TG_REQUIRE(tg_bn_fused_supported(rows, C, groups) && aligned16(x) && (y == nullptr || aligned16(y)),
               "tg_bn_train_fused: unsupported shape C=%d rows=%d groups=%d (see tg_bn_fused_supported) or unaligned pointers", C, rows, groups);
    hipLaunchKernelGGL(bn_small_train_kernel, dim3(1), dim3(BN_SMALL_THREADS), 0, (hipStream_t)stream, x, y, rows / groups, C, groups, mean, rstd,
                       running_mean, running_var, num_batches_tracked, gamma, beta, act_slope, eps, momentum, repeats);
    return check_launch("tg_bn_train_fused");
}

extern "C" int tg_bn_train_stats(const float* x, int32_t rows, int32_t C, int32_t groups, double* ws, float* mean, float* rstd,
                                 float* running_mean, float* running_var, int64_t* num_batches_tracked, float eps,
                                 float momentum, int32_t repeats, void* stream) {
    TG_REQUIRE(x && ws && mean && rstd && repeats >= 1, "tg_bn_train_stats: null pointer / repeats < 1");
    TG_REQUIRE(C > 0 && C <= 256 && groups > 0 && rows > 0 && rows % groups == 0, "tg_bn_train_stats: C=%d (<=256), rows=%d, groups=%d", C, rows, groups);
    hipStream_t s = (hipStream_t)stream;
    if (zero_async(ws, sizeof(double) * 2 * (size_t)groups * C, s)) return 1;
    const int rpg = rows / groups;
    const int rpi = 256 / C;
    int blocks = cdiv(rpg, rpi * 16);
    if (blocks > 1024) blocks = 1024;
    if (blocks < 1) blocks = 1;
// ... 16 lines not shown
    hipLaunchKernelGGL(bn_eval_stats_kernel, dim3(cdiv(C, 64)), dim3(64), 0, (hipStream_t)stream, running_mean, running_var, C, eps, mean, rstd);
    return check_launch("tg_bn_eval_stats");
}

extern "C" int tg_bn_apply(const float* x, float* y, int32_t rows, int32_t C, int32_t groups, const float* mean,
                           const float* rstd, const float* gamma, const float* beta, float act_slope, void* stream) {
    TG_REQUIRE(x && y && mean && rstd && gamma && beta, "tg_bn_apply: null pointer");
    TG_REQUIRE(rows > 0 && C > 0 && groups > 0 && rows % groups == 0, "tg_bn_apply: bad sizes");
    const bool vec = (C % 4 == 0) && aligned16(x) && aligned16(y);
    const long total = (long)rows * C;
    if (vec) hipLaunchKernelGGL((bn_apply_kernel<true>), dim3(ew_grid(total / 4, 256, 2)), dim3(256), 0, (hipStream_t)stream, x, y, (long)rows, C, rows / groups, mean, rstd, gamma, beta, act_slope);
    else     hipLaunchKernelGGL((bn_apply_kernel<false>), dim3(ew_grid(total, 256, 4)), dim3(256), 0, (hipStream_t)stream, x, y, (long)rows, C, rows / groups, mean, rstd, gamma, beta, act_slope);
    return check_launch("tg_bn_apply");
}

extern "C" int tg_bn_backward(const float* dy, const float* x, float* dx, int32_t rows, int32_t C, const float* mean,
                              const float* rstd, const float* gamma, const float* beta, float act_slope, double* ws,
                              float* dgamma, float* dbeta, void* stream) {
    TG_REQUIRE(dy && x && dx && mean && rstd && gamma && beta && ws, "tg_bn_backward: null pointer");
    TG_REQUIRE(rows > 0 && C > 0 && C <= 256, "tg_bn_backward: C=%d must be <= 256", C);
    hipStream_t s = (hipStream_t)stream;
    if (tg_bn_fused_supported(rows, C, 1) && aligned16(dy) && aligned16(x) && aligned16(dx)) {
        hipLaunchKernelGGL(bn_small_bwd_kernel, dim3(1), dim3(BN_SMALL_THREADS), 0, s, dy, x, dx, rows, C, mean, rstd, gamma, beta, act_slope,
                           dgamma, dbeta);
        return check_launch("tg_bn_backward(small)");
    }
    if (zero_async(ws, sizeof(double) * 2 * (size_t)C, s)) return 1;
    const int rpi = 256 / C;
    int blocks = cdiv(rows, rpi * 16);
    if (blocks > 1024) blocks = 1024;
    if (blocks < 1) blocks = 1;
    if (bn_vec_ok(C, (long)rows * C) && aligned16(dy) && aligned16(x) && aligned16(dx)) {
        const long total4 = (long)rows * C / 4;
        int vb = (int)((total4 + 256 * 8 - 1) / (256 * 8));
        if (vb > 2048) vb = 2048;
        if (vb < 1) vb = 1;
        hipLaunchKernelGGL(bn_bwd_reduce_vec_kernel, dim3(vb), dim3(256), 0, s, dy, x, (long)rows, C, mean, rstd, gamma, beta, act_slope, ws);
        hipLaunchKernelGGL(bn_bwd_apply_vec_kernel, dim3(vb), dim3(256), 0, s, dy, x, dx, (long)rows, C, mean, rstd, gamma, beta, act_slope, ws,
                           dgamma, dbeta);
        return check_launch("tg_bn_backward(vec)");
    }
    hipLaunchKernelGGL(bn_bwd_reduce_kernel, dim3(blocks), dim3(256), 0, s, dy, x, rows, C, mean, rstd, gamma, beta, act_slope, ws);
    hipLaunchKernelGGL(bn_bwd_apply_kernel, dim3(ew_grid((long)rows * C, 256, 4)), dim3(256), 0, s, dy, x, dx, (long)rows, C, mean, rstd,
                       gamma, beta, act_slope, ws, dgamma, dbeta);
    return check_launch("tg_bn_backward");
}

extern "C" int32_t tg_bn2_supported(int32_t rows_per_group, int32_t C) {
    return rows_per_group > 0 && bn_vec_ok(C, (long)rows_per_group * C) && 256 % C == 0;
}
static int bn2_parts(long rows_per_group, int C) {
    long p = (rows_per_group * C / 4 + 2047) / 2048;
    return (int)(p < 1 ? 1 : (p > 256 ? 256 : p));
}
constexpr int BN2_INLINE_PARTS = 32;
extern "C" int64_t tg_bn2_ws_doubles(int32_t rows_per_group, int32_t C, int32_t groups) {
    return tg_bn2_supported(rows_per_group, C) && groups > 0 ? (int64_t)groups * (bn2_parts(rows_per_group, C) + 1) * 2 * C : 0;
}
static const double* bn2_combine(double* ws, int P, int C, int groups, int* p_out, hipStream_t s) {
    if (P <= BN2_INLINE_PARTS) { *p_out = P; return ws; }
    double* tot = ws + (long)groups * P * 2 * C;
    hipLaunchKernelGGL(bn2_reduce_kernel, dim3(groups), dim3(256), 0, s, ws, P, C, tot);
    *p_out = 1;
    return tot;
}

extern "C" int tg_bn2_train(const float* x, float* y, int32_t rows_per_group, int32_t C, int32_t groups, double* ws, int64_t ws_doubles, float* mean,
                            float* rstd, float* running_mean, float* running_var, int64_t* num_batches_tracked, const float* gamma,
                            const float* beta, float act_slope, float eps, float momentum, int32_t repeats, void* stream) {
    TG_REQUIRE(x && ws && mean && rstd && groups > 0 && repeats >= 1 && (y == nullptr || (gamma && beta)), "tg_bn2_train: null pointer / bad counts");
    TG_REQUIRE(tg_bn2_supported(rows_per_group, C) && aligned16(x) && (y == nullptr || aligned16(y)), "tg_bn2_train: unsupported shape C=%d rows=%d (tg_bn2_supported) or unaligned pointers", C, rows_per_group);
    TG_REQUIRE(ws_doubles >= tg_bn2_ws_doubles(rows_per_group, C, groups), "tg_bn2_train: workspace too small");
    hipStream_t s = (hipStream_t)stream;
    const int P = bn2_parts(rows_per_group, C);
    hipLaunchKernelGGL(bn2_partial_kernel, dim3(P, groups), dim3(256), 0, s, x, (const float*)nullptr, (long)rows_per_group, C, (const float*)nullptr,
                       (const float*)nullptr, (const float*)nullptr, (const float*)nullptr, 1.f, ws, deterministic() ? 1 : 0);
    int Pa;
    const double* tot = bn2_combine(ws, P, C, groups, &Pa, s);
    hipLaunchKernelGGL(bn2_fwd_apply_kernel, dim3(P, groups), dim3(256), 0, s, x, y, (long)rows_per_group, C, groups, tot, Pa, mean, rstd, running_mean,
                       running_var, num_batches_tracked, gamma, beta, act_slope, eps, momentum, repeats);
    return check_launch("tg_bn2_train");
}

extern "C" int tg_bn2_backward(const float* dy, const float* x, float* dx, int32_t rows_per_group, int32_t C, int32_t groups, const float* mean,
                               const float* rstd, const float* gamma, const float* beta, float act_slope, double* ws, int64_t ws_doubles,
                               float* dgamma, float* dbeta, void* stream) {
    TG_REQUIRE(dy && x && dx && mean && rstd && gamma && beta && ws && groups > 0, "tg_bn2_backward: null pointer / bad counts");
    TG_REQUIRE(tg_bn2_supported(rows_per_group, C) && aligned16(dy) && aligned16(x) && aligned16(dx), "tg_bn2_backward: unsupported shape C=%d rows=%d or unaligned pointers", C, rows_per_group);
    TG_REQUIRE(ws_doubles >= tg_bn2_ws_doubles(rows_per_group, C, groups), "tg_bn2_backward: workspace too small");
    hipStream_t s = (hipStream_t)stream;
    const int P = bn2_parts(rows_per_group, C);
    hipLaunchKernelGGL(bn2_partial_kernel, dim3(P, groups), dim3(256), 0, s, x, dy, (long)rows_per_group, C, mean, rstd, gamma, beta, act_slope, ws, deterministic() ? 1 : 0);
    int Pa;
    const double* tot = bn2_combine(ws, P, C, groups, &Pa, s);
    hipLaunchKernelGGL(bn2_bwd_apply_kernel, dim3(P, groups), dim3(256), 0, s, dy, x, dx, (long)rows_per_group, C, groups, tot, Pa, mean, rstd, gamma, beta,
                       act_slope, dgamma, dbeta);
    return check_launch("tg_bn2_backward");
}
```

### gesture-generation-from-trimodal-context_amd/engine.py

```python

import os
import zlib

import torch

from . import layers as L
from . import ops, _lib
from .ops import Win
from .params import ParamSlab

WAV_CONVS = ((0, 16, 1, 5, 1600), (3, 32, 16, 6, 0), (6, 64, 32, 6, 0), (9, 32, 64, 6, 0))
WAV_KW = 15


class DeviceRNG:

    def __init__(self, seed, device):
        self.state = ops.new_rng_state(seed, device)
        self._sites = {}

    def site(self, name):
        sid = self._sites.get(name)
        if sid is None:
            sid = (zlib.crc32(name.encode()) & 0x7FFFFFFF) or 1
# ... 122 lines not shown
            elif ops.SPEAKER_FUSED:
                eps, draw = L.empty(Bs, 16, like=pre_seq), (self.rng.state, self.rng.site(f"{tag}.eps"))
            else:
                eps = ops.normal(L.empty(Bs, 16, like=pre_seq), self.rng.state, self.rng.site(f"{tag}.eps"))
            if ops.SPEAKER_FUSED:
                se, zc, mu, logvar, z = ops.speaker_fwd(P["speaker_embedding.0.weight"], vid.contiguous(), P["speaker_embedding.1.weight"],
                                                        P["speaker_embedding.1.bias"], P["speaker_mu.weight"], P["speaker_mu.bias"],
                                                        P["speaker_logvar.weight"], P["speaker_logvar.bias"], eps,
                                                        rep=in_data.view(Bs * T, in_size)[:, self.c_z:], T=T, draw=draw)
                z_in_place = True
            else:
                se = ops.embed_gather(P["speaker_embedding.0.weight"], vid.contiguous(), L.empty(Bs, 16, like=pre_seq))
                zc = L.linear_fwd(se, P["speaker_embedding.1.weight"], P["speaker_embedding.1.bias"])
                mu = L.linear_fwd(zc, P["speaker_mu.weight"], P["speaker_mu.bias"])
                logvar = L.linear_fwd(zc, P["speaker_logvar.weight"], P["speaker_logvar.bias"])
                z = ops.reparam_fwd(mu, logvar, eps, torch.empty_like(mu))
            tp.update(se=se, zc=zc, mu=mu, logvar=logvar, eps=eps, vid=vid)
        elif self.z_mode == "random":
            if inject is not None and f"{tag}.z" in inject:
                z = inject[f"{tag}.z"].contiguous()
            else:
                z = ops.normal(L.empty(Bs, 16, like=pre_seq), self.rng.state, self.rng.site(f"{tag}.z"))

        fork.join()
        L.prep_zone("post_join")
        flat_in = in_data.view(Bs * T, in_size)
        if not pre_in_place:
            ops.copy2d(pre_seq.contiguous().view(Bs * T, D + 1), flat_in[:, :D + 1])
        if z is not None and not z_in_place:
            ops.repeat_rows(z, flat_in[:, self.c_z:], Bs, T)

        y, gtape = L.gru_stack_fwd(in_data, P, "gru", self.n_layers, H, p_drop=self.p_drop, training=training, rng=self.rng,
                                   save=save, inject=inject, tag=tag, save_rows=save_rows)
        if ops.OUT_MLP_COMPOSED:
            w21, w21t, b21 = self._w21_early if self._w21_early is not None else \
                L.frozen(("w21", P["out.0.weight"].data_ptr()), lambda: ops.out_mlp_compose(P["out.0.weight"], P["out.0.bias"], P["out.2.weight"], P["out.2.bias"], dup=2))
            self._w21_early = None
            assert out_into is None or (tuple(out_into.shape) == (Bs, T, D) and out_into.is_contiguous())
            out = L.linear_fwd(y.view(Bs * T, 2 * H), w21, b21, out=None if out_into is None else out_into.view(Bs * T, D)).view(Bs, T, D)
            tp.update(in_text=in_text, gru=gtape, o=None, y_last=y, h1=None, w21t=w21t, in_size=in_size)
        else:
            o = ops.add_halves(y, L.empty(Bs * T, H, like=y))
            h1 = L.linear_fwd(o, P["out.0.weight"], P["out.0.bias"])
            out = L.linear_fwd(h1, P["out.2.weight"], P["out.2.bias"], out=None if out_into is None else out_into.view(Bs * T, D)).view(Bs, T, D)
            tp.update(in_text=in_text, gru=gtape, o=o, h1=h1, in_size=in_size)
        L.prep_zone("pre_join")
        return {"out": out, "z": z, "mu": mu, "logvar": logvar, "in_data": in_data, "tape": tp if save else None, "side_work_ran": self._side_work_ran}

    def _audio_fwd(self, P, Bf, in_audio, in_data, ca, tp, fork, training, groups, side_work=None, side_head=None):
        Bs, T, in_size = in_data.shape
        fe = "audio_encoder.feat_extractor"
        Ba = in_audio.shape[0]
        shared = Ba != Bs
        assert Ba == Bs or Ba * groups == Bs, (Ba, Bs, groups)
        x = in_audio.contiguous().view(Ba, -1, 1)
        wav = []
        fork.keep(x, in_data)
        fork.__enter__()
        if side_head is not None:
            assert fork.enabled, "side_head without a forked branch: the caller must check forks_in_forward()"
            side_head()
        for idx, Co, Ci, stride, pad in WAV_CONVS:
            if idx == 0 and L.wav_front_supported(P[f"{fe}.0.weight"]):
                y, st = L.wav_front_fwd(x.view(Ba, -1), P[f"{fe}.0.weight"], P[f"{fe}.0.bias"], P[f"{fe}.1.weight"], P[f"{fe}.1.bias"],
                                        Bf[f"{fe}.1.running_mean"], Bf[f"{fe}.1.running_var"], Bf[f"{fe}.1.num_batches_tracked"],
                                        stride=stride, pad=pad, training=training, groups=1 if shared else groups, act_slope=0.3,
                                        repeats=groups if shared else 1)
                wav.append((x, st, y.shape[1]))
                x = y
                continue
            wp = L.pack_conv_weight(P[f"{fe}.{idx}.weight"])
            last = idx == 9
            if last and shared:
                Lo = L.conv_out_len(x.shape[1], WAV_KW, stride, pad)
                assert Lo == T, f"audio length gives {Lo} frames, expected {T}"
                a_win = Win.conv(x, WAV_KW, stride=stride, pad=pad, rows_out=Lo)
                probs = []
                for g in range(groups):
                    o = in_data[g * Ba:(g + 1) * Ba, :, ca:ca + 32]
                    probs.append(dict(A=a_win, W=wp, bias=P[f"{fe}.{idx}.bias"], out=o, c_batch_stride=o.stride(0), c_row_stride=o.stride(1), c_rows_out=Lo))
                ops.gemm_nt_group(probs)
                wav.append((x, None, None))
                break
            out = in_data[:, :, ca:ca + 32] if last else None
            c = L.conv_fwd(x, wp, P[f"{fe}.{idx}.bias"], WAV_KW, stride=stride, pad=pad, out=out)
            if last:
                assert c.shape[1] == T, f"audio length gives {c.shape[1]} frames, expected {T}"
                wav.append((x, None, None))
                break
            y, st = L.bn_fwd(c, P[f"{fe}.{idx + 1}.weight"], P[f"{fe}.{idx + 1}.bias"], Bf[f"{fe}.{idx + 1}.running_mean"],
                             Bf[f"{fe}.{idx + 1}.running_var"], Bf[f"{fe}.{idx + 1}.num_batches_tracked"],
                             training=training, groups=1 if shared else groups, act_slope=0.3,
                             repeats=groups if shared else 1)
            wav.append((x, st, c.shape[1]))
            x = y
        if side_work is not None and fork.enabled:
            side_work()
            self._side_work_ran = True
        if fork.enabled and ops.OUT_MLP_COMPOSED and self.early_out_compose:
            self._w21_early = L.frozen(("w21", P["out.0.weight"].data_ptr()), lambda: ops.out_mlp_compose(P["out.0.weight"], P["out.0.bias"], P["out.2.weight"], P["out.2.bias"], dup=2))
        fork.__exit__(None, None, None)
        tp["wav"], tp["wav_shared"] = wav, shared

    def _text_fwd(self, P, in_text, in_data, tp, training, inject, tag, save=True, save_rows=None):
        Bs, T, in_size = in_data.shape
        te = "text_encoder"
        E = P[f"{te}.embedding.weight"].shape[1]
        if (training and self.tcn_drop_regen and Bs * T >= 8192 and E % 4 == 0 and P[f"{te}.embedding.weight"].data_ptr() % 16 == 0 and
                not (inject is not None and f"{tag}.emb_drop" in inject)):
            cur, emb_mask = ops.embed_gather_drop(P[f"{te}.embedding.weight"], in_text.contiguous().view(-1), L.empty(Bs, T, E, like=in_data), 0.1,
                                                  self.rng.state, self.rng.site(f"{tag}.emb_drop"))
        else:
            emb = ops.embed_gather(P[f"{te}.embedding.weight"], in_text.contiguous().view(-1), L.empty(Bs, T, E, like=in_data))
            cur, emb_mask = self._drop(f"{tag}.emb_drop", emb, 0.1, inject) if training else (emb, None)
        names = [f"{te}.tcn.network.{i}.{c}" for i in range(self.n_layers) for c in ("conv1", "conv2")]
        wps, wts = L.frozen(("tcn_wn", P[names[0] + ".weight_v"].data_ptr(), training),
                            lambda: ops.weight_norm_fwd_batch([P[n + ".weight_v"] for n in names], [P[n + ".weight_g"] for n in names], want_t=training))
        Co_w = wps.shape[1]
        w_pl = ops.split_planes(wps.view(len(names) * Co_w, wps.shape[2])) if (ops.GEMM_PLANES and Bs * T >= 8192) else None
        sites = [f"{tag}.tcn{i}.drop{ci + 1}" for i in range(self.n_layers) for ci in range(2)]
        masks = [None] * len(sites)
        if training:
            if inject is not None and all(sn in inject for sn in sites):
                masks = [inject[sn].contiguous() for sn in sites]
            elif self.p_drop > 0.0 and self.tcn_drop_regen and Bs * T >= 8192 and wps.shape[1] % 4 == 0:
                per = Bs * T * wps.shape[1]
                site = self.rng.site(f"{tag}.tcn.drop")
                masks = [inject[sn].contiguous() if (inject is not None and sn in inject) else
                         ops.Drop(self.rng.state, site, self.p_drop, (Bs, T, wps.shape[1]), index0=j * per) for j, sn in enumerate(sites)]
            elif self.p_drop > 0.0:
                drawn = ops.dropout_mask(L.empty(len(sites), Bs, T, wps.shape[1], like=in_data), self.p_drop, self.rng.state,
                                         self.rng.site(f"{tag}.tcn.drop"))
                masks = [inject[sn].contiguous() if (inject is not None and sn in inject) else drawn[j] for j, sn in enumerate(sites)]
        biases = [P[n + ".bias"] for n in names]
        if (training and wps.shape[1] == E and all(m is None or isinstance(m, ops.Drop) for m in masks)
                and ops.tcn_fused_takes(cur, w_pl, 2, self.n_layers, P[f"{te}.decoder.weight"], biases)):
            nb, Cc = self.n_layers, wps.shape[1]
            tape = tuple(L.empty(nb, Bs, T, Cc, like=cur) for _ in range(3)) if save else None
            drop = next((m for m in masks if m is not None), None)
            ops.tcn_fwd_fused(cur, w_pl, biases, P[f"{te}.decoder.weight"], P[f"{te}.decoder.bias"], in_data[:, :, self.c_text:self.c_text + 32],
                              p=drop.p if drop is not None else 0.0, state=drop.state if drop is not None else None,
                              site=drop.site if drop is not None else 0, save_rows=((0, Bs) if save_rows is None else save_rows) if save else None, tape=tape)
            tcn, x = [], cur
            for i in range(nb if save else 0):
                o0, o1, y = tape[0][i], tape[1][i], tape[2][i]
                tcn.append({"x": x, "d": 2 ** i, "in0": x, "wt0": wts[2 * i] if wts is not None else None, "o0": o0, "m0": masks[2 * i],
                            "in1": o0, "wt1": wts[2 * i + 1] if wts is not None else None, "o1": o1, "m1": masks[2 * i + 1], "y": y})
                x = y
            tp["tcn"], tp["emb_mask"], tp["text_x"] = tcn, emb_mask, (x if save else None)
            return
        tcn = []
        fuse_res = wps.shape[1] == cur.shape[2] and cur.is_contiguous() and ops.nt_ext_supported(
            Win.conv(cur, 2, pad=1, dil=1, rows_out=T), wps[0], cur, c_batch_stride=cur.stride(0), c_row_stride=cur.stride(1), c_rows_out=T)
        chain = (w_pl is not None and w_pl.kind == "h2" and fuse_res and cur.is_contiguous()
                 and ops.nt_kernel_plan([dict(A=Win.conv(cur, 2, pad=1, dil=1, rows_out=T), W=wps[0], bias=None, out=cur, c_batch_stride=cur.stride(0),
                                              c_row_stride=cur.stride(1), c_rows_out=T, w_planes=w_pl, a_rowmax=cur.view(-1))])[0] == 2)
        if chain:
            rmax = ops.zeros(1 + 2 * self.n_layers, Bs * T, device=cur.device)
            rm_in = ops.win_row_absmax(Win.conv(cur, 2, pad=1, dil=1, rows_out=T), out=rmax[0])
        for i in range(self.n_layers):
            d = 2 ** i
            blk = {"x": cur, "d": d}
            h = cur
            y = None
            for ci in range(2):
                j = 2 * i + ci
# ... 455 lines not shown
```

### gesture-generation-from-trimodal-context_amd/layers.py

```python
import os

import torch

from . import ops, _lib
from .ops import Win


def empty(*shape, like=None, device=None, dtype=torch.float32):
    return torch.empty(*shape, device=like.device if like is not None else device, dtype=dtype)


_FROZEN = None


class FrozenWeights:

    def __init__(self):
        self.memo = {}

    def __enter__(self):
        global _FROZEN
        self._prev, _FROZEN = _FROZEN, self.memo
        return self

# ... 318 lines not shown


def conv_dgrad_padded(dy, w, L_in, *, stride=1, pad=0, out=None, accumulate=False):
    B, Lo, Co = dy.shape
    _, Ci, kw = w.shape
    J = (kw + stride - 1) // stride
    packed = dgrad_pack(w, stride)
    if out is not None:
        assert tuple(out.shape) == (B, L_in, Ci) and out.is_contiguous()
    dx = out if out is not None else empty(B, L_in, Ci, like=w)
    probs = []
    for r in range(stride):
        nq = (L_in - r + stride - 1) // stride
        if nq <= 0:
            continue
        j0 = (r + pad) % stride
        probs.append(dict(A=Win.taps(dy, J, shift=(r + pad - j0) // stride, dil=-1, rows_out=nq), W=packed[j0], bias=None, out=dx[:, r:, :],
                          c_batch_stride=dx.stride(0), c_row_stride=stride * Ci, c_rows_out=nq, accumulate=bool(accumulate and out is not None)))
    ops.gemm_nt_group(probs)
    return dx


def conv_transpose_fwd(x, w, b, *, out=None):
    B, L, Ci = x.shape
    _, Co, kw = w.shape
    packed = dgrad_pack(w, 1)
    Lo = L + kw - 1
    if out is None:
        out = empty(B, Lo, Co, like=x)
    A = Win.taps(x, kw, shift=0, dil=-1, rows_out=Lo)
    ops.gemm_nt(A, packed[0], b, out, c_batch_stride=out.stride(0), c_row_stride=out.stride(1), c_rows_out=Lo)
    return out


def conv_transpose_bwd(dy, x, w, dW, db, need_dx=True):
    B, L, Ci = x.shape
    _, Co, kw = w.shape
    Lo = L + kw - 1
    A = Win.conv(dy, kw, rows_out=L)
    ops.gemm_tn(x.reshape(B * L, Ci), A, dW.view(Ci, -1), out_kw=kw)
    ops.colsum(dy.reshape(B * Lo, Co), db, accumulate=True)
    if not need_dx:
        return None
    return conv_fwd(dy, pack_conv_weight(w), None, kw, rows_out=L)


class BNState:
    __slots__ = ("mean", "rstd", "groups", "x", "slope")


def _eval_stats(running_mean, running_var, mean, rstd):
    def make():
        ops.bn_eval_stats(running_mean, running_var, mean, rstd)
        return mean, rstd
    return frozen(("bn_eval", running_mean.data_ptr(), running_var.data_ptr()), make)


def _a16(*ts):
    return all(t.data_ptr() % 16 == 0 for t in ts)


def bn_fwd(x, gamma, beta, running_mean, running_var, nbt, *, training, groups=1, act_slope=1.0, out=None, repeats=1):
    Cc = x.shape[-1]
    x2 = x.view(-1, Cc)
    st = BNState()
    g = groups if training else 1
    st.mean, st.rstd = empty(g, Cc, like=x), empty(g, Cc, like=x)
    st.groups, st.x, st.slope = g, x, act_slope
    y = torch.empty_like(x) if out is None else out
    a16 = _a16(x2, y)
    if training and a16 and x2.shape[0] % g == 0 and ops.bn2_supported(x2.shape[0] // g, Cc, g) and x2.is_contiguous():
        ops.bn2_train(x2, y.view(-1, Cc), g, st.mean, st.rstd, running_mean, running_var, nbt, gamma, beta, act_slope, repeats=repeats)
        return y, st
    if training and a16 and ops.bn_fused_supported(x2.shape[0], Cc, g):
        ops.bn_train_fused(x2, y.view(-1, Cc), g, st.mean, st.rstd, running_mean, running_var, nbt, gamma, beta, act_slope, repeats=repeats)
        return y, st
    if training:
        ws = torch.empty(2 * g * Cc, device=x.device, dtype=torch.float64)
        ops.bn_train_stats(x2, g, ws, st.mean, st.rstd, running_mean, running_var, nbt, repeats=repeats)
    else:
        st.mean, st.rstd = _eval_stats(running_mean, running_var, st.mean, st.rstd)
    ops.bn_apply(x2, y.view(-1, Cc), g, st.mean, st.rstd, gamma, beta, act_slope)
    return y, st


def bn_bwd(dy, st, gamma, beta, dgamma, dbeta, *, g0=0, ng=1, row0=0, out=None):
    Cc = dy.shape[-1]
    nb = dy.shape[0]
    assert nb % ng == 0
    per = nb // ng
    dy = dy.contiguous()
    dx = torch.empty_like(dy) if out is None else out
    assert dx.shape == dy.shape and dx.is_contiguous()
    rpg = dy[0].numel() // Cc * per
    x_all = st.x[row0:row0 + nb]
    if ops.bn2_supported(rpg, Cc, ng) and x_all.is_contiguous() and _a16(dy, x_all, dx):
        ops.bn2_backward(dy.view(-1, Cc), x_all.reshape(-1, Cc), dx.view(-1, Cc), ng, st.mean[g0:g0 + ng], st.rstd[g0:g0 + ng], gamma, beta, st.slope,
                         dgamma, dbeta)
        return dx
    ws = torch.empty(2 * Cc, device=dy.device, dtype=torch.float64)
    for g in range(ng):
        sl = slice(g * per, (g + 1) * per)
        x = st.x[row0 + g * per:row0 + (g + 1) * per]
        ops.bn_backward(dy[sl].reshape(-1, Cc), x.reshape(-1, Cc), dx[sl].view(-1, Cc), st.mean[g0 + g], st.rstd[g0 + g],
                        gamma, beta, st.slope, ws, dgamma, dbeta)
    return dx


class WavFrontState:
    __slots__ = ("mean", "rstd", "fstat", "gate", "groups", "slope", "stride", "pad", "T1", "words_per_clip")


def wav_front_supported(w):
    return ops.WAV_FUSED and tuple(w.shape) == (16, 1, 15)


def wav_front_fwd(audio, w, b, gamma, beta, running_mean, running_var, nbt, *, stride, pad, training, groups=1, act_slope=0.3, repeats=1):
    B, L = audio.shape
    T1 = conv_out_len(L, 15, stride, pad)
    g = groups if training else 1
    assert B % g == 0
    per = B // g
    st = WavFrontState()
    st.mean, st.rstd = empty(g, 16, like=audio), empty(g, 16, like=audio)
    st.groups, st.slope, st.stride, st.pad, st.T1 = g, act_slope, stride, pad, T1
    st.words_per_clip = 4 * ((T1 + 15) // 16)
    st.fstat = st.gate = None
    y = empty(B, T1, 16, like=audio)
    if training:
        st.fstat = torch.empty(g, 272, device=audio.device, dtype=torch.float64)
        st.gate = torch.empty(B * st.words_per_clip, device=audio.device, dtype=torch.int64)
        for q in range(g):
            ops.wav_front_stats(audio[q * per:(q + 1) * per], w, b, stride, pad, st.mean[q], st.rstd[q], running_mean, running_var, nbt,
                                st.fstat[q], repeats=repeats)
    else:
        st.mean, st.rstd = _eval_stats(running_mean, running_var, st.mean, st.rstd)
    for q in range(g):
        sl = slice(q * per, (q + 1) * per)
        ops.wav_front_apply(audio[sl], w, b, stride, pad, st.mean[q], st.rstd[q], gamma, beta, act_slope, y[sl],
                            st.gate[q * per * st.words_per_clip:(q + 1) * per * st.words_per_clip] if training else None)
    return y, st


def wav_front_bwd(dact, st, audio, w, b, gamma, dW, db, dgamma, dbeta, *, g0=0, row0=0):
    nb = dact.shape[0]
    wpc = st.words_per_clip
    ops.wav_front_backward(dact.contiguous(), st.gate[row0 * wpc:(row0 + nb) * wpc], audio[row0:row0 + nb], w, b, st.stride, st.pad,
                           st.mean[g0], st.rstd[g0], gamma, st.fstat[g0], st.slope, dW.view(-1) if dW is not None else None, db, dgamma, dbeta)


def wav_front_bwd_fused_supported(w2, stride2):
    return ops.WAV_FUSED_DGRAD and tuple(w2.shape) == (32, 16, 15) and stride2 == 6


def wav_front_bwd_fused(dc2, w2, st, audio, w, b, gamma, dW, db, dgamma, dbeta, *, g0=0, row0=0):
    nb = dc2.shape[0]
    wpc = st.words_per_clip
    ops.wav_front_backward_fused(dc2.contiguous(), w2, st.gate[row0 * wpc:(row0 + nb) * wpc], audio[row0:row0 + nb], w, b, st.stride, st.pad,
                                 st.mean[g0], st.rstd[g0], gamma, st.fstat[g0], st.slope, dW.view(-1) if dW is not None else None, db, dgamma, dbeta)


class GRUTape:
    __slots__ = ("x", "y", "save", "masks", "B", "T", "H", "xbound")


def gru_stack_fwd(x, P, prefix, n_layers, H, *, p_drop, training, rng=None, save=False, inject=None, tag="g", save_rows=None, drawn=None):
# ... 301 lines not shown
```

### gesture-generation-from-trimodal-context_amd/ops.py

```python
import ctypes as C

import contextlib
import os

import torch

from . import _lib
from ._lib import Window, call


def _stream():
    return C.c_void_p(torch.cuda.current_stream().cuda_stream)


def _f32(t, name="tensor"):
    if not (isinstance(t, torch.Tensor) and t.is_cuda and t.dtype == torch.float32):
        raise TypeError(f"{name}: expected a CUDA float32 tensor, got {type(t).__name__} "
                        f"{getattr(t, 'dtype', None)} {getattr(t, 'device', None)}")
    return t


def _p(t):
    return C.c_void_p(t.data_ptr()) if t is not None else C.c_void_p(0)

# ... 941 lines not shown
        raise ValueError("seq2seq_loss: output, target, d_output [B, T, P] of one shape; scalars >= 4 floats")
    B, T, P = output.shape
    if len(weights) != 3:
        raise ValueError(f"seq2seq_loss: weights must hold the three loss weights, got {len(weights)}")
    ws = torch.empty(3 * B, device=output.device, dtype=torch.float64)
    call("tg_seq2seq_loss", _p(output), _p(target), B, T, P, *[float(x) for x in weights], _p(ws), _p(scalars), _p(d_output), _stream())
    return scalars


def _f64_word(t, name):
    if not (isinstance(t, torch.Tensor) and t.is_cuda and t.dtype == torch.float64 and t.is_contiguous() and t.numel() >= 1):
        raise TypeError(f"{name}: expected a contiguous CUDA float64 tensor")
    return t


def grad_sumsq(g, total, ws=None):
    _flat(g, "g"); _f64_word(total, "total")
    if g.numel() == 0:
        return total
    if ws is None:
        ws = torch.empty(256, device=g.device, dtype=torch.float64)
    if _f64_word(ws, "ws").numel() < 256:
        raise ValueError("grad_sumsq: ws needs 256 float64")
    call("tg_sumsq_accumulate", _p(g), g.numel(), _p(ws), _p(total), _stream())
    return total


def clip_scale(total, max_norm, out):
    _f64_word(total, "total"); _flat(out, "out")
    if out.numel() < 2 or not max_norm > 0:
        raise ValueError("clip_scale: out needs 2 floats and max_norm must be positive")
    call("tg_clip_scale", _p(total), float(max_norm), _p(out), _stream())
    return out


def scale_by(x, scale):
    _flat(x, "x"); _flat(scale, "scale")
    if x.numel():
        call("tg_scale_by", _p(x), x.numel(), _p(scale), _stream())
    return x


def bn_train_stats(x2d, groups, ws, mean, rstd, running_mean, running_var, nbt, eps=1e-5, momentum=0.1, repeats=1):
    _flat(x2d, "x"); rows, Cc = x2d.shape
    assert ws.dtype == torch.float64 and ws.numel() >= 2 * groups * Cc and ws.is_cuda
    assert mean.numel() == groups * Cc == rstd.numel()
    assert nbt is None or (nbt.dtype == torch.int64 and nbt.is_cuda)
    call("tg_bn_train_stats", _p(x2d), rows, Cc, groups, _p(ws), _p(_flat(mean, "mean")), _p(_flat(rstd, "rstd")),
         _p(running_mean), _p(running_var), _p(nbt), float(eps), float(momentum), int(repeats), _stream())


def bn_fused_supported(rows, C, groups=1):
    return bool(_lib.load().tg_bn_fused_supported(int(rows), int(C), int(groups)))


def bn_train_fused(x2d, y2d, groups, mean, rstd, running_mean, running_var, nbt, gamma, beta, act_slope, eps=1e-5, momentum=0.1, repeats=1):
    _flat(x2d, "x"); _flat(y2d, "y"); rows, Cc = x2d.shape
    assert y2d.shape == x2d.shape and bn_fused_supported(rows, Cc, groups) and mean.numel() == groups * Cc == rstd.numel()
    assert gamma.numel() == Cc == beta.numel() and (nbt is None or (nbt.dtype == torch.int64 and nbt.is_cuda))
    call("tg_bn_train_fused", _p(x2d), _p(y2d), rows, Cc, groups, _p(_flat(mean, "mean")), _p(_flat(rstd, "rstd")), _p(running_mean),
         _p(running_var), _p(nbt), _p(_flat(gamma, "gamma")), _p(_flat(beta, "beta")), float(act_slope), float(eps), float(momentum),
         int(repeats), _stream())
    return y2d


BN2_MIN_ELEMS = 16384


def bn2_supported(rows_per_group, C, groups=1):
    return rows_per_group * C * groups >= BN2_MIN_ELEMS and bool(_lib.load().tg_bn2_supported(int(rows_per_group), int(C)))


def bn2_train(x2d, y2d, groups, mean, rstd, running_mean, running_var, nbt, gamma, beta, act_slope, eps=1e-5, momentum=0.1, repeats=1):
    _flat(x2d, "x"); rows, Cc = x2d.shape
    assert rows % groups == 0 and (y2d is None or (_flat(y2d, "y").shape == x2d.shape)) and mean.numel() == groups * Cc == rstd.numel()
    assert nbt is None or (nbt.dtype == torch.int64 and nbt.is_cuda)
    rpg = rows // groups
    ws = torch.empty(_lib.load().tg_bn2_ws_doubles(rpg, Cc, groups), device=x2d.device, dtype=torch.float64)
    call("tg_bn2_train", _p(x2d), _p(y2d), rpg, Cc, groups, _p(ws), ws.numel(), _p(_flat(mean, "mean")), _p(_flat(rstd, "rstd")), _p(running_mean),
         _p(running_var), _p(nbt), _p(gamma), _p(beta), float(act_slope), float(eps), float(momentum), int(repeats), _stream())
    return y2d


def bn2_backward(dy2d, x2d, dx2d, groups, mean, rstd, gamma, beta, act_slope, dgamma, dbeta):
    _flat(dy2d, "dy"); _flat(x2d, "x"); _flat(dx2d, "dx"); rows, Cc = x2d.shape
    assert dy2d.shape == x2d.shape == dx2d.shape and rows % groups == 0 and mean.numel() == groups * Cc == rstd.numel()
    assert mean.is_contiguous() and rstd.is_contiguous()
    rpg = rows // groups
    ws = torch.empty(_lib.load().tg_bn2_ws_doubles(rpg, Cc, groups), device=x2d.device, dtype=torch.float64)
    call("tg_bn2_backward", _p(dy2d), _p(x2d), _p(dx2d), rpg, Cc, groups, _p(mean), _p(rstd), _p(_flat(gamma, "gamma")), _p(_flat(beta, "beta")),
         float(act_slope), _p(ws), ws.numel(), _p(dgamma), _p(dbeta), _stream())
    return dx2d


def bn_eval_stats(running_mean, running_var, mean, rstd, eps=1e-5):
    Cc = running_mean.numel()
    call("tg_bn_eval_stats", _p(_flat(running_mean, "rm")), _p(_flat(running_var, "rv")), Cc, float(eps),
         _p(_flat(mean, "mean")), _p(_flat(rstd, "rstd")), _stream())


def bn_apply(x2d, y2d, groups, mean, rstd, gamma, beta, act_slope):
    _flat(x2d, "x"); _flat(y2d, "y"); rows, Cc = x2d.shape
    assert y2d.shape == x2d.shape and mean.numel() == groups * Cc and gamma.numel() == Cc == beta.numel()
    call("tg_bn_apply", _p(x2d), _p(y2d), rows, Cc, groups, _p(mean), _p(rstd), _p(_flat(gamma, "gamma")),
         _p(_flat(beta, "beta")), float(act_slope), _stream())
    return y2d


def bn_backward(dy2d, x2d, dx2d, mean, rstd, gamma, beta, act_slope, ws, dgamma, dbeta):
    _flat(dy2d, "dy"); _flat(x2d, "x"); _flat(dx2d, "dx"); rows, Cc = x2d.shape
    assert dy2d.shape == x2d.shape == dx2d.shape and mean.numel() >= Cc and ws.dtype == torch.float64 and ws.numel() >= 2 * Cc
    call("tg_bn_backward", _p(dy2d), _p(x2d), _p(dx2d), rows, Cc, _p(mean), _p(rstd), _p(gamma), _p(beta),
         float(act_slope), _p(ws), _p(dgamma), _p(dbeta), _stream())
    return dx2d


WAV_FUSED = True
WAV_FUSED_DGRAD = True
_wav_ws = {}


def _wav_scratch(dev):
    ws = _wav_ws.get(dev)
    if ws is None:
        ws = torch.empty(_lib.load().tg_wav_front_ws_doubles(), dtype=torch.float64, device=dev)
        _wav_ws[dev] = ws
    return ws


def _wav_geom(audio, w, bias, stride, pad):
    _f32(audio, "audio"); _flat(w, "w"); _flat(bias, "bias")
    assert audio.dim() == 2 and audio.stride(1) == 1, (audio.shape, audio.stride())
    B, L = audio.shape
    assert tuple(w.shape) == (16, 1, 15) and bias.numel() == 16, w.shape
    if (B - 1) * audio.stride(0) + L - 1 >= _room(audio):
        raise ValueError("wav_front: audio exceeds its tensor")
    T1 = (L + 2 * pad - 15) // stride + 1
    return B, L, T1


def wav_front_stats(audio, w, bias, stride, pad, mean, rstd, running_mean, running_var, nbt, fstat, eps=1e-5, momentum=0.1, repeats=1):
    B, L, T1 = _wav_geom(audio, w, bias, stride, pad)
    ws = _wav_scratch(audio.device)
    assert mean.numel() == 16 == rstd.numel() and fstat.dtype == torch.float64 and fstat.numel() >= _lib.load().tg_wav_front_fstat_doubles()
    assert nbt is None or (nbt.dtype == torch.int64 and nbt.is_cuda)
    call("tg_wav_front_stats", _p(audio), audio.stride(0), B, L, _p(w), _p(bias), int(stride), int(pad), T1, _p(ws), ws.numel(),
         _p(_flat(mean, "mean")), _p(_flat(rstd, "rstd")), _p(running_mean), _p(running_var), _p(nbt), _p(fstat), float(eps), float(momentum),
         int(repeats), _stream())


def wav_front_apply(audio, w, bias, stride, pad, mean, rstd, gamma, beta, act_slope, y, gate=None):
    B, L, T1 = _wav_geom(audio, w, bias, stride, pad)
    _flat(y, "y"); assert tuple(y.shape) == (B, T1, 16), (y.shape, B, T1)
    assert mean.numel() == 16 == rstd.numel() == gamma.numel() == beta.numel()
    if gate is not None:
        assert gate.dtype == torch.int64 and gate.is_cuda and gate.is_contiguous() and gate.numel() >= _lib.load().tg_wav_front_gate_words(B, T1)
    call("tg_wav_front_apply", _p(audio), audio.stride(0), B, L, _p(w), _p(bias), int(stride), int(pad), T1, _p(_flat(mean, "mean")),
         _p(_flat(rstd, "rstd")), _p(_flat(gamma, "gamma")), _p(_flat(beta, "beta")), float(act_slope), _p(y), _p(gate), _stream())
    return y


def wav_front_backward(dact, gate, audio, w, bias, stride, pad, mean, rstd, gamma, fstat, act_slope, dW, dbias, dgamma, dbeta):
    B, L, T1 = _wav_geom(audio, w, bias, stride, pad)
    _flat(dact, "dact"); assert tuple(dact.shape) == (B, T1, 16), (dact.shape, B, T1)
    assert gate.dtype == torch.int64 and gate.is_cuda and gate.is_contiguous() and gate.numel() >= _lib.load().tg_wav_front_gate_words(B, T1)
    assert fstat.dtype == torch.float64 and fstat.is_cuda and fstat.numel() >= _lib.load().tg_wav_front_fstat_doubles()
# ... 1122 lines not shown
```

### include/trimodal_hip.h

```cpp
#ifndef TRIMODAL_HIP_H
#define TRIMODAL_HIP_H

#include <stdint.h>

#ifdef __cplusplus
extern "C" {
#endif

#define TG_ABI_VERSION 11

int tg_version(void);

int tg_set_deterministic(int32_t on);
int tg_get_deterministic(void);
int tg_set_tn_workgroup_cap(int32_t n);
int tg_get_tn_workgroup_cap(void);
const char* tg_last_error(void);

int tg_set_math_mode(int32_t mode);
int tg_get_math_mode(void);

typedef struct tg_window {
    const float* ptr;
    int64_t batch_stride;
// ... 74 lines not shown
    const float* y_colmax;
    const float* a_colmax;
} tg_gemm_tn_problem;
int tg_gemm_tn_group(const tg_gemm_tn_problem* problems, int32_t n, void* stream);
int32_t tg_gemm_tn_kernel_plan(const tg_gemm_tn_problem* problems, int32_t n);
int tg_gemm_tn(const float* dY, int64_t ldy, const tg_window* A, float* dW, int64_t ldw, int32_t M, int32_t N,
               int32_t out_kw, float* dbias, float* ws, int64_t ws_floats, void* stream);

int tg_colsum(const float* X, int64_t ldx, int32_t M, int32_t N, float* out, int32_t accumulate, void* stream);

int tg_gru_forward(const float* gi, int64_t gi_dir_stride, const float* w_hh_fwd, const float* w_hh_rev,
                   const float* b_hh_fwd, const float* b_hh_rev, float* y, float* save, int64_t save_dir_stride,
                   int32_t B, int32_t T, int32_t H, void* stream);

int tg_gru_backward(const float* dy, const float* y, const float* save, int64_t save_dir_stride,
                    const float* w_hh_t_fwd, const float* w_hh_t_rev, float* dgi, float* dgh, int64_t dg_dir_stride,
                    float* dh_scratch, int32_t B, int32_t T, int32_t H, void* stream);

int tg_gru_h64_forward(const float* gi, int64_t gi_dir_stride, const float* w_hh_fwd, const float* w_hh_rev,
                       const float* b_hh_fwd, const float* b_hh_rev, float* y, float* save, int64_t save_dir_stride,
                       const float* drop_mask, float* y_drop, int32_t B, int32_t T, void* stream);
int tg_gru_h64_backward(const float* dy, const float* dy_mask, const float* y, const float* save, int64_t save_dir_stride,
                        const float* w_hh_t_fwd, const float* w_hh_t_rev, float* dgi, float* dgh, int64_t dg_dir_stride,
                        int32_t B, int32_t T, void* stream);

int32_t tg_gru_cluster_supported(int32_t B, int32_t H);
int64_t tg_gru_cluster_ws_bytes(int32_t B, int32_t H);
int32_t tg_gru_cluster_fused_dropout(void);
int tg_gru_forward_cluster(const float* gi, int64_t gi_dir_stride, const float* w_hh_fwd, const float* w_hh_rev,
                           const float* b_hh_fwd, const float* b_hh_rev, float* y, float* save, int64_t save_dir_stride,
                           const float* drop_mask, float* y_drop, void* ws, int64_t ws_bytes, int32_t B, int32_t T, int32_t H, void* stream);
int tg_gru_forward_cluster_rows(const float* gi, int64_t gi_dir_stride, const float* w_hh_fwd, const float* w_hh_rev,
                                const float* b_hh_fwd, const float* b_hh_rev, float* y, float* save, int64_t save_dir_stride,
                                const float* drop_mask, float* y_drop, void* ws, int64_t ws_bytes, int32_t B, int32_t T, int32_t H,
                                int32_t save_row0, int32_t save_rows, void* stream);

int32_t tg_gru_vec_supported(int32_t B, int32_t H);
int64_t tg_gru_vec_ws_bytes(int32_t H);
int32_t tg_gru_vec_ws_header_bytes(void);
int tg_gru_forward_vec(const float* gi, int64_t gi_dir_stride, const float* w_hh_fwd, const float* w_hh_rev, const float* b_hh_fwd,
                       const float* b_hh_rev, float* y, void* ws, int64_t ws_bytes, int32_t B, int32_t T, int32_t H, void* stream);
int tg_gru_vec1_supported(int32_t B, int32_t H, int32_t* supported);
int tg_gru_forward_vec1(const float* gi, const float* w_hh, const float* b_hh, float* y, void* ws, int64_t ws_bytes, int32_t B, int32_t T,
                        int32_t H, void* stream);
int tg_gru_vec_const_supported(int32_t B, int32_t H, int32_t n_dir, int32_t* supported);
int tg_gru_forward_vec_const(const float* gi, int64_t gi_dir_stride, const float* w_hh_fwd, const float* w_hh_rev, const float* b_hh_fwd,
                             const float* b_hh_rev, float* y, void* ws, int64_t ws_bytes, int32_t B, int32_t T, int32_t H, int32_t n_dir,
                             void* stream);

int32_t tg_gru_cluster_bwd_supported(int32_t B, int32_t H);
int64_t tg_gru_cluster_bwd_ws_bytes(int32_t B, int32_t H);
int tg_gru_backward_cluster(const float* dy, const float* dy_mask, const float* y, const float* save, int64_t save_dir_stride,
                            const float* w_hh_t_fwd, const float* w_hh_t_rev, float* dgi, float* dgh, int64_t dg_dir_stride,
                            void* ws, int64_t ws_bytes, int32_t B, int32_t T, int32_t H, void* stream);
int tg_gru_backward_cluster_stats(const float* dy, const float* dy_mask, const float* y, const float* save, int64_t save_dir_stride,
                                  const float* w_hh_t_fwd, const float* w_hh_t_rev, float* dgi, float* dgh, int64_t dg_dir_stride,
                                  void* ws, int64_t ws_bytes, int32_t B, int32_t T, int32_t H, float* gi_rowmax, int64_t rowmax_dir_stride,
                                  float* gi_colmax, float* gh_colmax, void* stream);

int tg_bn_train_stats(const float* x, int32_t rows, int32_t C, int32_t groups, double* ws, float* mean, float* rstd,
                      float* running_mean, float* running_var, int64_t* num_batches_tracked, float eps,
                      float momentum, int32_t repeats, void* stream);
int32_t tg_bn_fused_supported(int32_t rows, int32_t C, int32_t groups);
int tg_bn_train_fused(const float* x, float* y, int32_t rows, int32_t C, int32_t groups, float* mean, float* rstd,
                      float* running_mean, float* running_var, int64_t* num_batches_tracked, const float* gamma,
                      const float* beta, float act_slope, float eps, float momentum, int32_t repeats, void* stream);
int tg_bn_eval_stats(const float* running_mean, const float* running_var, int32_t C, float eps, float* mean,
                     float* rstd, void* stream);
int tg_bn_apply(const float* x, float* y, int32_t rows, int32_t C, int32_t groups, const float* mean,
                const float* rstd, const float* gamma, const float* beta, float act_slope, void* stream);
int tg_bn_backward(const float* dy, const float* x, float* dx, int32_t rows, int32_t C, const float* mean,
                   const float* rstd, const float* gamma, const float* beta, float act_slope, double* ws,
                   float* dgamma, float* dbeta, void* stream);

int32_t tg_bn2_supported(int32_t rows_per_group, int32_t C);
int64_t tg_bn2_ws_doubles(int32_t rows_per_group, int32_t C, int32_t groups);
int tg_bn2_train(const float* x, float* y, int32_t rows_per_group, int32_t C, int32_t groups, double* ws, int64_t ws_doubles, float* mean,
                 float* rstd, float* running_mean, float* running_var, int64_t* num_batches_tracked, const float* gamma,
                 const float* beta, float act_slope, float eps, float momentum, int32_t repeats, void* stream);
int tg_bn2_backward(const float* dy, const float* x, float* dx, int32_t rows_per_group, int32_t C, int32_t groups, const float* mean,
                    const float* rstd, const float* gamma, const float* beta, float act_slope, double* ws, int64_t ws_doubles,
                    float* dgamma, float* dbeta, void* stream);

int32_t tg_d_preconv_fwd_supported(int32_t Bs, int32_t groups);
int64_t tg_d_preconv_ws_bytes(int32_t Bs);
int tg_d_preconv_fwd(const float* poses, const float* w1, const float* b1, const float* gamma1, const float* beta1, const float* w2,
                     const float* b2, const float* gamma2, const float* beta2, const float* w3, const float* b3, float* c1, float* y1,
                     float* c2, float* y2, float* c3, float* mean1, float* rstd1, float* mean2, float* rstd2, float* running_mean1,
                     float* running_var1, int64_t* nbt1, float* running_mean2, float* running_var2, int64_t* nbt2, void* ws,
                     int64_t ws_bytes, int32_t Bs, int32_t groups, float eps, float momentum, void* stream);

int tg_d_preconv_bwd(const float* dc3, const float* poses, const float* c1, const float* y1, const float* c2, const float* y2,
                     const float* mean1, const float* rstd1, const float* mean2, const float* rstd2, const float* w1, const float* w2,
                     const float* w3, const float* gamma1, const float* gamma2, float* dw1, float* db1, float* dgamma1, float* dbeta1,
                     float* dw2, float* db2, float* dgamma2, float* dbeta2, float* dw3, float* db3, float* dposes,
                     int32_t dposes_accumulate, void* ws, int64_t ws_bytes, int32_t nb, int32_t groups, void* stream);

int tg_speaker_fwd(const float* table, const int64_t* vid, int32_t n_rows, const float* w1, const float* b1, const float* wmu, const float* bmu,
                   const float* wlv, const float* blv, float* eps, float* se, float* zc, float* mu, float* logvar, float* z,
                   int32_t B, float* rep, int64_t rep_ld, int32_t T, const uint64_t* rng_state, uint32_t site, void* stream);
int32_t tg_speaker_bwd_max_rows(void);
int tg_speaker_bwd(const float* dz, const float* d_mu_in, const float* d_logvar_in, const float* logvar, const float* eps, const float* zc,
                   const float* se, const int64_t* vid, int32_t n_rows, const float* w1, const float* wmu, const float* wlv, float* dw1,
                   float* db1, float* dwmu, float* dbmu, float* dwlv, float* dblv, float* dtable, int32_t nb, void* stream);

int tg_out_mlp_compose(const float* w1, const float* b1, const float* w2, const float* b2, int32_t H, int32_t Hm, int32_t D, int32_t dup,
                       float* w21, float* w21t, float* b21, void* stream);
int tg_out_mlp_param_grads(const float* P, const float* s, const float* w1, const float* b1, const float* w2, int32_t H, int32_t Hm, int32_t D,
                           int32_t dup, float* dw1, float* db1, float* dw2, float* db2, void* stream);

int64_t tg_wav_front_ws_doubles(void);
int64_t tg_wav_front_fstat_doubles(void);
int64_t tg_wav_front_gate_words(int32_t B, int32_t T1);
int tg_wav_front_stats(const float* audio, int64_t audio_stride, int32_t B, int32_t L, const float* w, const float* bias, int32_t stride,
                       int32_t pad, int32_t T1, double* ws, int64_t ws_doubles, float* mean, float* rstd, float* running_mean,
                       float* running_var, int64_t* num_batches_tracked, double* fstat, float eps, float momentum, int32_t repeats,
                       void* stream);
int tg_wav_front_apply(const float* audio, int64_t audio_stride, int32_t B, int32_t L, const float* w, const float* bias, int32_t stride,
                       int32_t pad, int32_t T1, const float* mean, const float* rstd, const float* gamma, const float* beta, float act_slope,
                       float* y, uint64_t* gate, void* stream);
int tg_wav_front_backward(const float* dact, const uint64_t* gate, const float* audio, int64_t audio_stride, int32_t B, int32_t L, const float* w,
                          const float* bias, int32_t stride, int32_t pad, int32_t T1, const float* mean, const float* rstd, const float* gamma,
                          const double* fstat, float act_slope, double* ws, int64_t ws_doubles, float* dW, float* dbias, float* dgamma,
                          float* dbeta, void* stream);

int tg_wav_front_backward_fused(const float* dc2, int32_t T2, const float* w2, const uint64_t* gate, const float* audio, int64_t audio_stride,
                                int32_t B, int32_t L, const float* w, const float* bias, int32_t stride, int32_t pad, int32_t T1,
                                const float* mean, const float* rstd, const float* gamma, const double* fstat, float act_slope, double* ws,
                                int64_t ws_doubles, float* dW, float* dbias, float* dgamma, float* dbeta, void* stream);

int64_t tg_wav_conv2_wgrad_ws_floats(void);
int tg_wav_conv2_wgrad(const float* dc2, const float* act, int32_t B, int32_t T1, int32_t T2, float* ws, int64_t ws_floats, float* dW2,
                       float* db2, void* stream);

int tg_add_relu(const float* a, const float* b, float* y, int64_t n, void* stream);
int tg_act_mask_bwd2(const float* dy, const float* y, const float* o, const float* mask, float slope, float* dsum, float* dc, int64_t n, void* stream);
int tg_act_mask_bwd(const float* dy, const float* y, const float* mask, float slope, float* dx, int64_t n,
                    void* stream);
int tg_act_mask_bwd_drop(const float* dy, const float* y, float p, const uint64_t* rng_state, uint32_t site, int64_t index0, float slope,
                         float* dx, int64_t n, void* stream);
int tg_act_mask_bwd2_drop(const float* dy, const float* y, const float* o, float p, const uint64_t* rng_state, uint32_t site, int64_t index0,
                          float slope, float* dsum, float* dc, int64_t n, void* stream);
int tg_mul(const float* x, const float* mask, float* y, int64_t n, void* stream);
int tg_zero(void* p, int64_t bytes, void* stream);
int tg_axpy(const float* x, float* y, float alpha, int32_t accumulate, int64_t n, void* stream);
int tg_copy2d(const float* src, int64_t lds, float* dst, int64_t ldd, int32_t rows, int32_t cols,
              int32_t accumulate, void* stream);
int tg_repeat_rows(const float* src, int64_t lds, float* dst, int64_t ldd, int32_t B, int32_t T, int32_t cols,
                   void* stream);
int tg_sum_rows(const float* src, int64_t lds, float* dst, int64_t ldd, int32_t B, int32_t T, int32_t cols,
                int32_t accumulate, void* stream);
int tg_add_halves(const float* y, float* o, int32_t M, int32_t H, void* stream);
int tg_sum_parts(const float* parts, int64_t stride, int32_t n_parts, float* out, int64_t n, void* stream);
int tg_narrow8_pair(const float* a0, const float* a1, const float* w0, const float* w1, float* out, int32_t M, int32_t K, void* stream);
int tg_dup_halves(const float* d_o, float* dy, int32_t M, int32_t H, void* stream);
int tg_make_pre_seq(const float* target, float* pre, int32_t B, int32_t T, int32_t D, int32_t n_pre, void* stream);
int tg_assemble_batch(const float* audio_raw, const int64_t* audio_off, const float* vec_raw, const int64_t* vec_off, const int64_t* word_idx,
                      const double* word_onset, const int32_t* n_words, const double* times, const int32_t* n_ext, const int64_t* vid_in, int32_t B, int32_t Wmax,
                      int32_t n_poses, int32_t pose_floats, int32_t audio_len, int32_t remove_word_timing, int64_t* out_text, float* out_audio,
                      float* out_vec, int64_t* out_vid, void* stream);
int tg_embed_gather(const float* table, const int64_t* idx, float* out, int32_t n_idx, int32_t D, int32_t n_rows,
                    void* stream);
int tg_embed_gather_drop(const float* table, const int64_t* idx, float* out, int32_t n_idx, int32_t D, int32_t n_rows, float p,
                         const uint64_t* rng_state, uint32_t site, void* stream);
int tg_tcn_fwd_fused(const float* x0, const void* w_planes, int64_t w_plane_stride, int32_t w_rows, const float* w_inv, const float* const* biases,
                     const float* dec_w, const float* dec_b, const uint64_t* rng_state, uint32_t site, float p, int32_t clips, int32_t T, int32_t C,
// ... 200 lines not shown
```

Measured before the change: 30570 clips/s.

## Fuse BatchNorm statistics into audio conv GEMM epilogue with self-finalizing apply

```diff
diff --git a/gesture-generation-from-trimodal-context_amd/_lib.py b/gesture-generation-from-trimodal-context_amd/_lib.py
--- a/gesture-generation-from-trimodal-context_amd/_lib.py
+++ b/gesture-generation-from-trimodal-context_amd/_lib.py
@@ -67,6 +67,8 @@
     "tg_bn_train_fused": [P, P, I32, I32, I32, P, P, P, P, P, P, P, F32, F32, F32, I32, P],
     "tg_bn_apply": [P, P, I32, I32, I32, P, P, P, P, F32, P],
     "tg_bn2_train": [P, P, I32, I32, I32, P, I64, P, P, P, P, P, P, P, F32, F32, F32, I32, P],
+    "tg_gemm_nt_bn": [C.POINTER(NtProblem), I32, I32, P, I64, P, P],
+    "tg_bn2_apply_parts": [P, P, I32, I32, I32, P, I32, I64, I32, P, P, P, P, P, P, P, F32, F32, F32, I32, P],
     "tg_bn2_backward": [P, P, P, I32, I32, I32, P, P, P, P, F32, P, I64, P, P, P],
     "tg_bn_backward": [P, P, P, I32, I32, P, P, P, P, F32, P, P, P, P],
     "tg_wav_front_stats": [P, I64, I32, I32, P, P, I32, I32, I32, P, I64, P, P, P, P, P, P, F32, F32, I32, P],
diff --git a/gesture-generation-from-trimodal-context_amd/csrc/common.hpp b/gesture-generation-from-trimodal-context_amd/csrc/common.hpp
--- a/gesture-generation-from-trimodal-context_amd/csrc/common.hpp
+++ b/gesture-generation-from-trimodal-context_amd/csrc/common.hpp
@@ -94,6 +94,8 @@
     int h2;
     float* c_rmax;
     float* c2_rmax;
+    double* bn_part;
+    int bn_rpg, bn_groups, bn_P;
 };
 
 struct NtGroup {
diff --git a/gesture-generation-from-trimodal-context_amd/csrc/gemm.hip b/gesture-generation-from-trimodal-context_amd/csrc/gemm.hip
--- a/gesture-generation-from-trimodal-context_amd/csrc/gemm.hip
+++ b/gesture-generation-from-trimodal-context_amd/csrc/gemm.hip
@@ -45,9 +45,10 @@
     }
 }
 
-template <bool VEC, int WM, int WN, int NT_RING, int KS = 1>
+template <bool VEC, int WM, int WN, int NT_RING, int KS = 1, bool STATS = false>
 __global__ __launch_bounds__(256) void gemm_nt_kernel(const NtGroup g) {
     static_assert(KS == 1 || (KS == 4 && WM == 1 && WN == 1 && VEC), "K split: one tile per workgroup, vectorised path");
+    static_assert(!STATS || (WM == 4 && WN == 1 && KS == 1), "STATS: one column tile per workgroup, its four waves stacked over the rows");
     const int pi = group_find(g, blockIdx.x);
     const NtProb& pr = g.p[pi];
     const Win A = pr.A;
@@ -66,7 +67,7 @@
     const int lid = xcd_chunked_id(blockIdx.x - g.wg_begin[pi], g.wg_begin[pi + 1] - g.wg_begin[pi]);
     const int m_base = (lid / n_nt) * (WM * 32) + wm * 32;
     const int n_base = (lid % n_nt) * (WN * 32) + wn * 32;
-    if (m_base >= M || n_base >= N) return;
+    if (!STATS && (m_base >= M || n_base >= N)) return;
     const int kslice = KS > 1 ? ((A.K + 16 * KS - 1) / (16 * KS)) * 16 : A.K;
     const int K_beg = KS > 1 ? wave * kslice : 0;
     const int K = KS > 1 ? (A.K < K_beg + kslice ? A.K : K_beg + kslice) : A.K;
@@ -228,7 +229,42 @@
                 if (mul) v *= mv[mt][i][nt];
                 if (accumulate) v += cv[mt][i][nt];
                 if (okc[mt][i][nt]) C[off[mt][i][nt]] = v;
-            }
+                if constexpr (STATS) acc[mt][nt][i] = v;
+            }
+    if constexpr (STATS) {
+        __shared__ double sred[4][2][32];
+        const int P = pr.bn_P, rpg = pr.bn_rpg;
+        for (int gq = 0; gq < pr.bn_groups; ++gq) {
+            const int lo = gq * rpg, hi = lo + rpg;
+            double s[2] = {0.0, 0.0}, ss[2] = {0.0, 0.0};
+#pragma unroll
+            for (int mt = 0; mt < 2; ++mt)
+#pragma unroll
+                for (int i = 0; i < 4; ++i) {
+                    const int row = m_base + mt * 16 + kq * 4 + i;
+                    const bool in = row >= lo && row < hi && row < M;
+#pragma unroll
+                    for (int nt = 0; nt < 2; ++nt) {
+                        const double v = in ? (double)acc[mt][nt][i] : 0.0;
+                        s[nt] += v;
+                        ss[nt] += v * v;
+                    }
+                }
+#pragma unroll
+            for (int nt = 0; nt < 2; ++nt) {
+                s[nt] += __shfl_xor(s[nt], 16, 64);  ss[nt] += __shfl_xor(ss[nt], 16, 64);
+                s[nt] += __shfl_xor(s[nt], 32, 64);  ss[nt] += __shfl_xor(ss[nt], 32, 64);
+                if (kq == 0) { sred[wave][0][nt * 16 + r16] = s[nt]; sred[wave][1][nt * 16 + r16] = ss[nt]; }
+            }
+            __syncthreads();
+            if (threadIdx.x < 64) {
+                const int which = threadIdx.x >> 5, col = threadIdx.x & 31;
+                const double tsum = ((sred[0][which][col] + sred[1][which][col]) + sred[2][which][col]) + sred[3][which][col];
+                if (col < N) pr.bn_part[(((long)gq * P + lid) * 2 + which) * N + col] = tsum;
+            }
+            __syncthreads();
+        }
+    }
 }
 
 template <int TM, int TN, int BK = 16>
@@ -661,6 +697,18 @@
     return wg;
 }
 
+int tg_gemm_nt_split_bn_parts(NtGroup& g);
+static int nt_bn_parts(NtGroup& g) {
+    const NtProb& p = g.p[0];
+    if (g.n != 1 || p.mul || p.drop_state || p.accumulate || nt_has_ext(p) || p.c_rmax || p.c2_rmax || !nt_vec(p) || p.N % 4 != 0) return 0;
+    const int fam = nt_family(p);
+    if (fam == 0) return use_split_path() ? tg_gemm_nt_split_bn_parts(g) : 0;
+    if (fam != 1 || p.b_seg_k != p.A.K) return 0;
+    const int wgs = (cdiv(p.M, 128) * cdiv(p.N, 32) + 7) / 8 * 8;
+    if (wgs < 256 && p.A.K >= 256) return 0;
+    return wgs;
+}
+
 static int nt_launch(NtGroup& g, hipStream_t s) {
     const int fam = nt_family(g.p[0]);
     bool vec = true;
@@ -706,6 +754,12 @@
             else hipLaunchKernelGGL((gemm_nt_kernel<true, 1, 1, 2, 4>), grid4, dim3(256), 0, s, g);
             return check_launch("tg_gemm_nt");
         }
+        if (g.p[0].bn_part) {
+            TG_REQUIRE(nt_bn_parts(g) == wgs && g.p[0].bn_P == wgs, "tg_gemm_nt_bn: plan mismatch");
+            if (deep) hipLaunchKernelGGL((gemm_nt_kernel<true, 4, 1, 4, 1, true>), grid, dim3(256), 0, s, g);
+            else      hipLaunchKernelGGL((gemm_nt_kernel<true, 4, 1, 1, 1, true>), grid, dim3(256), 0, s, g);
+            return check_launch("tg_gemm_nt_bn");
+        }
         if (fam == 1) {
             if (vec && deep) hipLaunchKernelGGL((gemm_nt_kernel<true, 4, 1, 4>), grid, dim3(256), 0, s, g);
             else if (vec)    hipLaunchKernelGGL((gemm_nt_kernel<true, 4, 1, 1>), grid, dim3(256), 0, s, g);
@@ -737,6 +791,7 @@
     p.Bpl = nullptr; p.bpl_plane = 0; p.b_slab_rows = 0; p.b_row0 = 0;
     p.h2 = 0; p.a_scale = nullptr; p.a_rmax = nullptr; p.b_inv = nullptr; p.a_rmax_div = 1;
     p.c_rmax = q.c_rowmax; p.c2_rmax = q.c2_rowmax;
+    p.bn_part = nullptr; p.bn_rpg = p.bn_groups = p.bn_P = 0;
     TG_REQUIRE(!q.c2_rowmax || q.C2, "tg_gemm_nt: c2_rowmax without C2 (problem %d)", idx);
     if (q.b_planes) {
         const int64_t kp = ((int64_t)q.A.K + 31) / 32 * 32;
@@ -801,6 +856,27 @@
     for (int i = 0; i < n; ++i)
         if (int e = nt_fill(g.p[i], problems[i], i)) return e;
     for (int i = n; i < TG_MAX_GROUP; ++i) g.p[i] = g.p[0];
+    return nt_launch(g, (hipStream_t)stream);
+}
+
+extern "C" int tg_gemm_nt_bn(const tg_gemm_nt_problem* problem, int32_t rows_per_group, int32_t groups, double* part, int64_t part_doubles,
+                             int32_t* parts, void* stream) {
+    TG_REQUIRE(problem && parts, "tg_gemm_nt_bn: null pointer");
+    *parts = 0;
+    TG_REQUIRE(rows_per_group > 0 && groups > 0 && groups <= 64 && (int64_t)rows_per_group * groups == problem->M,
+               "tg_gemm_nt_bn: rows_per_group=%d * groups=%d must be M=%d (groups <= 64)", rows_per_group, groups, problem->M);
+    NtGroup g;
+    g.n = 1;
+    if (int e = nt_fill(g.p[0], *problem, 0)) return e;
+    for (int i = 1; i < TG_MAX_GROUP; ++i) g.p[i] = g.p[0];
+    const int P = nt_bn_parts(g);
+    *parts = P;
+    if (!part || P == 0) {
+        TG_REQUIRE(!part, "tg_gemm_nt_bn: this product's kernel has no statistics epilogue (M=%d N=%d K=%d): ask with part == NULL first", problem->M, problem->N, problem->A.K);
+        return 0;
+    }
+    TG_REQUIRE(part_doubles >= (int64_t)groups * P * 2 * problem->N, "tg_gemm_nt_bn: partial-row buffer too small (%ld doubles)", (long)part_doubles);
+    for (int i = 0; i < TG_MAX_GROUP; ++i) { g.p[i].bn_part = part; g.p[i].bn_rpg = rows_per_group; g.p[i].bn_groups = groups; g.p[i].bn_P = P; }
     return nt_launch(g, (hipStream_t)stream);
 }
 
diff --git a/gesture-generation-from-trimodal-context_amd/csrc/gemm_split.hip b/gesture-generation-from-trimodal-context_amd/csrc/gemm_split.hip
--- a/gesture-generation-from-trimodal-context_amd/csrc/gemm_split.hip
+++ b/gesture-generation-from-trimodal-context_amd/csrc/gemm_split.hip
@@ -7,7 +7,7 @@
 
 constexpr int SP_LD = 32;
 
-template <int TM, int TN, int SPLITS, int DB, int RING = 1, int OCC = 1, int ABL = 0, bool FAST = false>
+template <int TM, int TN, int SPLITS, int DB, int RING = 1, int OCC = 1, int ABL = 0, bool FAST = false, bool STATS = false>
 __global__ __launch_bounds__(256, OCC) void gemm_nt_split_kernel(const NtGroup g) {
     const int pi = group_find(g, blockIdx.x);
     const NtProb& pr = g.p[pi];
@@ -274,11 +274,43 @@
                 }
                 if (accumulate) v += cv[u];
                 if (ok[u]) *reinterpret_cast<f32x4*>(C + o[u]) = v;
+                if constexpr (STATS) *reinterpret_cast<f32x4*>(&ct[rl * CLD + 4 * c4]) = v;
                 if (res) {
                     f32x4 w = v + rv[u];
 #pragma unroll
                     for (int q = 0; q < 4; ++q) w[q] = act_fn(w[q], slope2);
                     if (ok[u]) *reinterpret_cast<f32x4*>(C2 + o[u]) = w;
+                }
+            }
+        }
+        if constexpr (STATS) {
+            constexpr int SL = 256 / BN;
+            __shared__ double sred[2][SL * BN];
+            const int P = pr.bn_P, rpg = pr.bn_rpg;
+            const int c = t % BN, sl = t / BN;
+            for (int gq = 0; gq < pr.bn_groups; ++gq) {
+                __syncthreads();
+                int r_lo = gq * rpg - m0, r_hi = r_lo + rpg;
+                r_lo = r_lo < 0 ? 0 : r_lo;
+                r_hi = r_hi > BM ? BM : r_hi;
+                r_hi = r_hi > M - m0 ? M - m0 : r_hi;
+                if (sl < SL) {
+                    double a = 0.0, b = 0.0;
+                    for (int r = r_lo + sl; r < r_hi; r += SL) {
+                        const double v = (double)ct[r * CLD + c];
+                        a += v;
+                        b += v * v;
+                    }
+                    sred[0][t] = a; sred[1][t] = b;
+                }
+                __syncthreads();
+                if (t < BN && n0 + t < N) {
+                    double a = 0.0, b = 0.0;
+#pragma unroll
+                    for (int q = 0; q < SL; ++q) { a += sred[0][q * BN + t]; b += sred[1][q * BN + t]; }
+                    double* orow = pr.bn_part + (((long)gq * P + lid) * 2) * N;
+                    orow[n0 + t] = a;
+                    orow[N + n0 + t] = b;
                 }
             }
         }
@@ -537,6 +569,21 @@
 bool tg_gemm_nt_mw_eligible(NtGroup& g, int* tm, int* tn);
 int tg_gemm_nt_mw_launch(NtGroup& g, int tm, int tn, int splits, hipStream_t s);
 
+static bool nt_fast_on() {
+    static const int fast_on = [] { const char* e = getenv("TG_NT_FAST"); return e ? atoi(e) : 1; }();
+    return fast_on != 0 && g_math_mode == 0;
+}
+
+int tg_gemm_nt_split_bn_parts(NtGroup& g) {
+    int tm = 0, tn = 0;
+    if (tg_gemm_nt_mw_eligible(g, &tm, &tn)) return 0;
+    const NtProb& p = g.p[0];
+    if (!p.vec_c || !nt_fast_on() || !nt_fast_ok(p)) return 0;
+    const SplitTile tl = split_pick_tile(p.M, p.N);
+    if (p.N > 32 * tl.tn) return 0;
+    return cdiv(p.M, 32 * tl.tm);
+}
+
 int tg_gemm_nt_split_launch(NtGroup& g, hipStream_t s) {
     {
         int tm = 0, tn = 0;
@@ -574,9 +621,18 @@
         else if (tl.tm == 2 && tl.tn == 3) TG_SPLIT(2, 3, SP_, 1);      \
         else TG_SPLIT(2, 2, SP_, 1);                                    \
     } while (0)
-    static const int fast_on = [] { const char* e = getenv("TG_NT_FAST"); return e ? atoi(e) : 1; }();
-    bool fast = fast_on != 0 && g_math_mode == 0;
+    bool fast = nt_fast_on();
     for (int i = 0; i < g.n && fast; ++i) fast = nt_fast_ok(g.p[i]);
+    if (g.p[0].bn_part) {
+        TG_REQUIRE(fast && g.n == 1 && g.p[0].n_nt == 1 && g.p[0].vec_c && g.p[0].bn_P == cdiv(g.p[0].M, bm), "tg_gemm_nt_bn: plan mismatch");
+#define TG_FAST_BN(TM_, TN_, DB_, R_, O_) hipLaunchKernelGGL((gemm_nt_split_kernel<TM_, TN_, 3, DB_, R_, O_, 0, true, true>), grid, dim3(256), 0, s, g)
+        if (tl.tm == 4 && tl.tn == 3) TG_FAST_BN(4, 3, 0, 1, 3);
+        else if (tl.tm == 4 && tl.tn == 2) TG_FAST_BN(4, 2, 0, 1, 4);
+        else if (tl.tm == 2 && tl.tn == 3) TG_FAST_BN(2, 3, 1, 1, 1);
+        else TG_FAST_BN(2, 2, 1, 1, 1);
+#undef TG_FAST_BN
+        return check_launch("tg_gemm_nt_bn(split)");
+    }
     if (fast) {
 #define TG_FAST(TM_, TN_, DB_, R_, O_) hipLaunchKernelGGL((gemm_nt_split_kernel<TM_, TN_, 3, DB_, R_, O_, 0, true>), grid, dim3(256), 0, s, g)
         if (tl.tm == 4 && tl.tn == 3) TG_FAST(4, 3, 0, 1, 3);
diff --git a/gesture-generation-from-trimodal-context_amd/csrc/norm.hip b/gesture-generation-from-trimodal-context_amd/csrc/norm.hip
--- a/gesture-generation-from-trimodal-context_amd/csrc/norm.hip
+++ b/gesture-generation-from-trimodal-context_amd/csrc/norm.hip
@@ -430,12 +430,13 @@
     }
 }
 
+template <int UNR = 8>
 __device__ __forceinline__ void bn2_totals(const double* __restrict__ part, int g, int P, int C, double (*tot)[256], double (*sl)[256]) {
     const int S = 256 / C;
     const int c = threadIdx.x % C, sidx = threadIdx.x / C;
     double a = 0.0, b = 0.0;
     if (sidx < S) {
-#pragma unroll 8
+#pragma unroll UNR
         for (int p = sidx; p < P; p += S) {
             const double* o = part + (((long)g * P + p) * 2) * C;
             a += o[c];
@@ -526,6 +527,67 @@
     }
 }
 
+__global__ __launch_bounds__(256) void bn2_fwd_apply_self_kernel(const float* __restrict__ x, float* __restrict__ y, long rows_per_group, int C, int groups,
+                                                                 const double* __restrict__ part, int P, float* __restrict__ mean, float* __restrict__ rstd,
+                                                                 float* __restrict__ rmean, float* __restrict__ rvar, int64_t* __restrict__ nbt,
+                                                                 const float* __restrict__ gamma, const float* __restrict__ beta, float slope, float eps,
+                                                                 float momentum, int repeats) {
+    __shared__ double tot[2][256], sl[2][256];
+    __shared__ float s_mean[256], s_rstd[256];
+    const int g = blockIdx.y;
+    const double n = (double)rows_per_group;
+    const bool stats_wg = blockIdx.x == 0 && g == 0;
+    float rm = 0.f, rv = 0.f;
+    if (stats_wg && (int)threadIdx.x < C) { rm = rmean ? rmean[threadIdx.x] : 0.f; rv = rvar ? rvar[threadIdx.x] : 0.f; }
+    const int g_end = stats_wg ? groups : g + 1;
+    for (int gg = g; gg < g_end; ++gg) {
+        bn2_totals<32>(part, gg, P, C, tot, sl);
+        if ((int)threadIdx.x < C) {
+            const int c = threadIdx.x;
+            const double m = tot[0][c] / n;
+            double var = tot[1][c] / n - m * m;
+            if (var < 0.0) var = 0.0;
+            if (gg == g) {
+                const float mf = (float)m, rs = (float)(1.0 / sqrt(var + (double)eps));
+                s_mean[c] = mf; s_rstd[c] = rs;
+                if (blockIdx.x == 0) { mean[g * C + c] = mf; rstd[g * C + c] = rs; }
+            }
+            if (stats_wg) {
+                const double unbiased = rows_per_group > 1 ? var * n / (n - 1.0) : var;
+                for (int q = 0; q < repeats; ++q) {
+                    rm = (1.f - momentum) * rm + momentum * (float)m;
+                    rv = (1.f - momentum) * rv + momentum * (float)unbiased;
+                }
+            }
+        }
+        __syncthreads();
+    }
+    if (stats_wg) {
+        if ((int)threadIdx.x < C) {
+            if (rmean) rmean[threadIdx.x] = rm;
+            if (rvar) rvar[threadIdx.x] = rv;
+        }
+        if (threadIdx.x == 0 && nbt) *nbt += (int64_t)groups * repeats;
+    }
+    if (y == nullptr) return;
+    const long total4 = rows_per_group * C / 4;
+    const long i0 = (long)blockIdx.x * 256 + threadIdx.x, step = (long)gridDim.x * 256;
+    const int c0 = (int)((i0 * 4) % C);
+    float mu[4], rs[4], ga[4], be[4];
+#pragma unroll
+    for (int q = 0; q < 4; ++q) { mu[q] = s_mean[c0 + q]; rs[q] = s_rstd[c0 + q]; ga[q] = gamma[c0 + q]; be[q] = beta[c0 + q]; }
+    const f32x4* x4 = reinterpret_cast<const f32x4*>(x) + (long)g * total4;
+    f32x4* y4 = reinterpret_cast<f32x4*>(y) + (long)g * total4;
+#pragma unroll 4
+    for (long i = i0; i < total4; i += step) {
+        const f32x4 v = x4[i];
+        f32x4 o;
+#pragma unroll
+        for (int q = 0; q < 4; ++q) o[q] = act_fn((v[q] - mu[q]) * rs[q] * ga[q] + be[q], slope);
+        y4[i] = o;
+    }
+}
+
 __global__ __launch_bounds__(256) void bn2_bwd_apply_kernel(const float* __restrict__ dy, const float* __restrict__ x, float* __restrict__ dx,
                                                             long rows_per_group, int C, int groups, const double* __restrict__ part, int P,
                                                             const float* __restrict__ mean, const float* __restrict__ rstd,
@@ -708,6 +770,27 @@
     return check_launch("tg_bn2_train");
 }
 
+extern "C" int tg_bn2_apply_parts(const float* x, float* y, int32_t rows_per_group, int32_t C, int32_t groups, double* part, int32_t parts,
+                                  int64_t part_doubles, int32_t self_finalize, float* mean, float* rstd, float* running_mean, float* running_var,
+                                  int64_t* num_batches_tracked, const float* gamma, const float* beta, float act_slope, float eps, float momentum,
+                                  int32_t repeats, void* stream) {
+    TG_REQUIRE(x && part && mean && rstd && groups > 0 && parts > 0 && repeats >= 1 && (y == nullptr || (gamma && beta)), "tg_bn2_apply_parts: null pointer / bad counts");
+    TG_REQUIRE(tg_bn2_supported(rows_per_group, C) && aligned16(x) && (y == nullptr || aligned16(y)), "tg_bn2_apply_parts: unsupported shape C=%d rows=%d (tg_bn2_supported) or unaligned pointers", C, rows_per_group);
+    TG_REQUIRE(part_doubles >= (int64_t)groups * (parts + (self_finalize ? 0 : 1)) * 2 * C, "tg_bn2_apply_parts: partial-row buffer too small");
+    hipStream_t s = (hipStream_t)stream;
+    const int G = bn2_parts(rows_per_group, C);
+    if (self_finalize) {
+        hipLaunchKernelGGL(bn2_fwd_apply_self_kernel, dim3(G, groups), dim3(256), 0, s, x, y, (long)rows_per_group, C, groups, (const double*)part, parts, mean, rstd,
+                           running_mean, running_var, num_batches_tracked, gamma, beta, act_slope, eps, momentum, repeats);
+        return check_launch("tg_bn2_apply_parts");
+    }
+    double* tot = part + (long)groups * parts * 2 * C;
+    hipLaunchKernelGGL(bn2_reduce_kernel, dim3(groups), dim3(256), 0, s, (const double*)part, parts, C, tot);
+    hipLaunchKernelGGL(bn2_fwd_apply_kernel, dim3(G, groups), dim3(256), 0, s, x, y, (long)rows_per_group, C, groups, (const double*)tot, 1, mean, rstd, running_mean,
+                       running_var, num_batches_tracked, gamma, beta, act_slope, eps, momentum, repeats);
+    return check_launch("tg_bn2_apply_parts(reduce)");
+}
+
 extern "C" int tg_bn2_backward(const float* dy, const float* x, float* dx, int32_t rows_per_group, int32_t C, int32_t groups, const float* mean,
                                const float* rstd, const float* gamma, const float* beta, float act_slope, double* ws, int64_t ws_doubles,
                                float* dgamma, float* dbeta, void* stream) {
diff --git a/gesture-generation-from-trimodal-context_amd/engine.py b/gesture-generation-from-trimodal-context_amd/engine.py
--- a/gesture-generation-from-trimodal-context_amd/engine.py
+++ b/gesture-generation-from-trimodal-context_amd/engine.py
@@ -228,6 +228,15 @@
                 ops.gemm_nt_group(probs)
                 wav.append((x, None, None))
                 break
+            if not last and training:
+                r = L.conv_bn_fwd(x, wp, P[f"{fe}.{idx}.bias"], WAV_KW, P[f"{fe}.{idx + 1}.weight"], P[f"{fe}.{idx + 1}.bias"],
+                                  Bf[f"{fe}.{idx + 1}.running_mean"], Bf[f"{fe}.{idx + 1}.running_var"], Bf[f"{fe}.{idx + 1}.num_batches_tracked"],
+                                  stride=stride, pad=pad, groups=1 if shared else groups, act_slope=0.3, repeats=groups if shared else 1)
+                if r is not None:
+                    c, y, st = r
+                    wav.append((x, st, c.shape[1]))
+                    x = y
+                    continue
             out = in_data[:, :, ca:ca + 32] if last else None
             c = L.conv_fwd(x, wp, P[f"{fe}.{idx}.bias"], WAV_KW, stride=stride, pad=pad, out=out)
             if last:
diff --git a/gesture-generation-from-trimodal-context_amd/layers.py b/gesture-generation-from-trimodal-context_amd/layers.py
--- a/gesture-generation-from-trimodal-context_amd/layers.py
+++ b/gesture-generation-from-trimodal-context_amd/layers.py
@@ -424,6 +424,31 @@
         st.mean, st.rstd = _eval_stats(running_mean, running_var, st.mean, st.rstd)
     ops.bn_apply(x2, y.view(-1, Cc), g, st.mean, st.rstd, gamma, beta, act_slope)
     return y, st
+
+
+def conv_bn_fwd(x, w_packed, b, kw, gamma, beta, running_mean, running_var, nbt, *, stride=1, pad=0, groups=1, act_slope=1.0, repeats=1):
+    B, L, _ = x.shape
+    Lo = conv_out_len(L, kw, stride, pad)
+    Co = w_packed.shape[0]
+    rows = B * Lo
+    if not ops.AUDIO_BN_EPI or rows % groups or not ops.bn2_supported(rows // groups, Co, groups):
+        return None
+    rpg = rows // groups
+    c = empty(B, Lo, Co, like=x)
+    A = Win.conv(x, kw, stride=stride, pad=pad, rows_out=Lo)
+    addr = dict(c_batch_stride=c.stride(0), c_row_stride=c.stride(1), c_rows_out=Lo)
+    parts = ops.gemm_nt_bn_parts(A, w_packed, b, c, rpg, groups, **addr)
+    if parts == 0 or parts > ops.AUDIO_BN_EPI_MAX_PARTS or not _a16(c):
+        return None
+    part = ops.bn_parts_buffer(parts, Co, groups, x.device)
+    ops.gemm_nt_bn(A, w_packed, b, c, rpg, groups, part, **addr)
+    st = BNState()
+    st.mean, st.rstd = empty(groups, Co, like=x), empty(groups, Co, like=x)
+    st.groups, st.x, st.slope = groups, c, act_slope
+    y = torch.empty_like(c)
+    ops.bn2_apply_parts(c.view(-1, Co), y.view(-1, Co), groups, part, parts, st.mean, st.rstd, running_mean, running_var, nbt, gamma, beta, act_slope,
+                        repeats=repeats, self_finalize=ops.AUDIO_BN_SELF)
+    return c, y, st
 
 
 def bn_bwd(dy, st, gamma, beta, dgamma, dbeta, *, g0=0, ng=1, row0=0, out=None):
diff --git a/gesture-generation-from-trimodal-context_amd/ops.py b/gesture-generation-from-trimodal-context_amd/ops.py
--- a/gesture-generation-from-trimodal-context_amd/ops.py
+++ b/gesture-generation-from-trimodal-context_amd/ops.py
@@ -1047,6 +1047,44 @@
     return y2d
 
 
+AUDIO_BN_EPI = os.environ.get("TG_AUDIO_BN_EPI", "1") != "0"
+AUDIO_BN_EPI_MAX_PARTS = int(os.environ.get("TG_AUDIO_BN_EPI_MAX_PARTS", "512"))
+AUDIO_BN_SELF = os.environ.get("TG_AUDIO_BN_SELF", "1") != "0"
+
+
+def gemm_nt_bn_parts(A: Win, W, bias, out, rows_per_group, groups, **kw):
+    q = _nt_problem(A, W, bias, out, **kw)
+    if q.M != rows_per_group * groups:
+        return 0
+    parts = C.c_int32(0)
+    call("tg_gemm_nt_bn", C.byref(q), int(rows_per_group), int(groups), None, 0, C.c_void_p(C.addressof(parts)), _stream())
+    return parts.value
+
+
+def bn_parts_buffer(parts, Cc, groups, device):
+    return torch.empty(groups * (parts + 1) * 2 * Cc, device=device, dtype=torch.float64)
+
+
+def gemm_nt_bn(A: Win, W, bias, out, rows_per_group, groups, part, **kw):
+    q = _nt_problem(A, W, bias, out, **kw)
+    assert part.dtype == torch.float64 and part.is_cuda and part.is_contiguous() and q.M == rows_per_group * groups
+    parts = C.c_int32(0)
+    call("tg_gemm_nt_bn", C.byref(q), int(rows_per_group), int(groups), _p(part), part.numel(), C.c_void_p(C.addressof(parts)), _stream())
+    return parts.value
+
+
+def bn2_apply_parts(x2d, y2d, groups, part, parts, mean, rstd, running_mean, running_var, nbt, gamma, beta, act_slope, eps=1e-5, momentum=0.1,
+                    repeats=1, self_finalize=True):
+    _flat(x2d, "x"); rows, Cc = x2d.shape
+    assert rows % groups == 0 and (y2d is None or (_flat(y2d, "y").shape == x2d.shape)) and mean.numel() == groups * Cc == rstd.numel()
+    assert nbt is None or (nbt.dtype == torch.int64 and nbt.is_cuda)
+    assert part.dtype == torch.float64 and part.is_cuda and part.is_contiguous()
+    call("tg_bn2_apply_parts", _p(x2d), _p(y2d), rows // groups, Cc, groups, _p(part), int(parts), part.numel(), int(bool(self_finalize)),
+         _p(_flat(mean, "mean")), _p(_flat(rstd, "rstd")), _p(running_mean), _p(running_var), _p(nbt), _p(gamma), _p(beta), float(act_slope),
+         float(eps), float(momentum), int(repeats), _stream())
+    return y2d
+
+
 def bn2_backward(dy2d, x2d, dx2d, groups, mean, rstd, gamma, beta, act_slope, dgamma, dbeta):
     _flat(dy2d, "dy"); _flat(x2d, "x"); _flat(dx2d, "dx"); rows, Cc = x2d.shape
     assert dy2d.shape == x2d.shape == dx2d.shape and rows % groups == 0 and mean.numel() == groups * Cc == rstd.numel()
diff --git a/include/trimodal_hip.h b/include/trimodal_hip.h
--- a/include/trimodal_hip.h
+++ b/include/trimodal_hip.h
@@ -180,6 +180,13 @@
                     const float* rstd, const float* gamma, const float* beta, float act_slope, double* ws, int64_t ws_doubles,
                     float* dgamma, float* dbeta, void* stream);
 
+int tg_gemm_nt_bn(const tg_gemm_nt_problem* problem, int32_t rows_per_group, int32_t groups, double* part, int64_t part_doubles, int32_t* parts,
+                  void* stream);
+int tg_bn2_apply_parts(const float* x, float* y, int32_t rows_per_group, int32_t C, int32_t groups, double* part, int32_t parts,
+                       int64_t part_doubles, int32_t self_finalize, float* mean, float* rstd, float* running_mean, float* running_var,
+                       int64_t* num_batches_tracked, const float* gamma, const float* beta, float act_slope, float eps, float momentum,
+                       int32_t repeats, void* stream);
+
 int32_t tg_d_preconv_fwd_supported(int32_t Bs, int32_t groups);
 int64_t tg_d_preconv_ws_bytes(int32_t Bs);
 int tg_d_preconv_fwd(const float* poses, const float* w1, const float* b1, const float* gamma1, const float* beta1, const float* w2,
```

New measurement: 30570 clips/s, median of 2. About the same (-0.0%).
